# SuperScientificSoftwareLaboratory/TileSpMV

Measured on AMD Instinct MI355X. Metric: fp64 SpMV GFLOP/s (y = A*x, tiled format), higher is better.
Workload: dtype f64; 1 GPU; laplacian4096; rows=16777216, cols=16777216, nnz=83869696, partition=tile-row blocks, nnz-balanced, 1 rank(s), y_combine=none, tiles=5234176, x_panel_merge=0, x_slice_passes=0

## Files before the change

include/tilespmv.h:

```cpp
#ifndef TILESPMV_H_
#define TILESPMV_H_

#include <stddef.h>
#include <stdint.h>

#ifdef __cplusplus
extern "C" {
#endif

#ifndef MAT_VAL_TYPE
#define MAT_VAL_TYPE double
#endif
#ifndef MAT_PTR_TYPE
#define MAT_PTR_TYPE int
#endif

#define TILESPMV_BLOCK_SIZE 16
#define TILESPMV_COO_NNZ_TH 12
#define TILESPMV_PREFETCH_SMEM_TH 4

enum {
    TILESPMV_FMT_CSR = 0,
    TILESPMV_FMT_COO = 1,
    TILESPMV_FMT_ELL = 2,
// ... 87 lines not shown
                      const MAT_PTR_TYPE *csrRowPtr, const int *csrColIdx, const MAT_VAL_TYPE *csrVal,
                      const char *source_mtx);
int tilespmv_csr_load(const char *path, int *m, int *n, MAT_PTR_TYPE *nnz, int *isSymmetric,
                      MAT_PTR_TYPE **csrRowPtr, int **csrColIdx, MAT_VAL_TYPE **csrVal,
                      const char *source_mtx);
int mmio_allinone_cached(int *m, int *n, MAT_PTR_TYPE *nnz, int *isSymmetric, MAT_PTR_TYPE **csrRowPtr,
                         int **csrColIdx, MAT_VAL_TYPE **csrVal, char *filename, const char *cache_path,
                         int *from_cache);
int tilespmv_mtx_write(const char *path, int m, int n, MAT_PTR_TYPE nnz, const MAT_PTR_TYPE *csrRowPtr,
                       const int *csrColIdx, const MAT_VAL_TYPE *csrVal);


void call_tilespmv_hip(char *filename, Tile_matrix *matrix, int *ptroffset1, int *ptroffset2,
                       int rowblkblock, unsigned int *blkcoostylerowidx,
                       int *blkcoostylerowidx_colstart, int *blkcoostylerowidx_colstop, int rowA,
                       int colA, MAT_PTR_TYPE nnzA, MAT_PTR_TYPE *csrRowPtrA, int *csrColIdxA,
                       MAT_VAL_TYPE *csrValA, MAT_VAL_TYPE alpha, MAT_VAL_TYPE *x,
                       MAT_VAL_TYPE *y, MAT_VAL_TYPE *y_golden);

#define TILESPMV_Y_SHARDED 0
#define TILESPMV_Y_ALLGATHER 1
#define TILESPMV_Y_ALLREDUCE 2
int call_tilespmv_hip_multi(char *filename, Tile_matrix *matrix, int *ptroffset1, int *ptroffset2,
                             int rowblkblock, unsigned int *blkcoostylerowidx,
                             int *blkcoostylerowidx_colstart, int *blkcoostylerowidx_colstop,
                             int rowA, int colA, MAT_PTR_TYPE nnzA, MAT_PTR_TYPE *csrRowPtrA,
                             int *csrColIdxA, MAT_VAL_TYPE *csrValA, MAT_VAL_TYPE alpha,
                             MAT_VAL_TYPE *x, MAT_VAL_TYPE *y, MAT_VAL_TYPE *y_golden, int ngpus,
                             const int *device_ids, int y_combine_mode);

typedef struct tilespmv_plan tilespmv_plan;

#define TILESPMV_COO_AUTO 0
#define TILESPMV_COO_IN_TILE 1
#define TILESPMV_COO_FALLBACK 2

#define TILESPMV_DENSE_AUTO 0
#define TILESPMV_DENSE_MFMA 1
#define TILESPMV_DENSE_VALU 2

#define TILESPMV_KERNEL_AUTO 0
#define TILESPMV_KERNEL_DIRECT 1
#define TILESPMV_KERNEL_STREAM 2

#define TILESPMV_KNOB_DEFAULT (-1)
typedef struct {
    unsigned size;
    int coo_mode;
    int dense_mode;
    int kernel;
    int tilerow_begin;
    int tilerow_end;
    int autotune;
    int entry_mode;
    int entry_ordered;
    int strip_cost;
    int split_above;
    int split_cap;
    int xcd_remap;
    int xcd_chunk;
    int csr_split;
    int fix_inline;
    int coo_cost;
    int coo_heavy_min;
    int coo_piece;
    int strip_even;
    int wg_strips;
    int x_window;
    int x_stride1;
    int x_stride2;
    int mv_native;
    int mv_xcd_chunk;
    int lds_pad;
    int y_store;
    int desc_dict;
    int nt_stream;
    int x_panel_kb;
    int x_panel_merge;
    int placement_tries;
    int x_slice_passes;
    int deterministic;
    int absorb;
    int value_narrow;
    int reserved[1];
} tilespmv_plan_options;
void tilespmv_plan_options_init(tilespmv_plan_options *opts);
const char *tilespmv_plan_options_layout(void);

int tilespmv_plan_create(tilespmv_plan **plan, const Tile_matrix *matrix, int rowA, int colA,
                         MAT_PTR_TYPE nnzA, const tilespmv_plan_options *opts);
void tilespmv_plan_destroy(tilespmv_plan *plan);

int Tile_create_device(Tile_matrix *matrix, int rowA, int colA, MAT_PTR_TYPE nnzA, const MAT_PTR_TYPE *csrRowPtrA,
                       const int *csrColIdxA, const MAT_VAL_TYPE *csrValA, unsigned flags);
int tilespmv_plan_create_from_csr(tilespmv_plan **plan, int rowA, int colA, MAT_PTR_TYPE nnzA, const MAT_PTR_TYPE *csrRowPtrA,
                                  const int *csrColIdxA, const MAT_VAL_TYPE *csrValA, unsigned create_flags,
                                  const tilespmv_plan_options *opts);
int tilespmv_plan_create_from_device_csr(tilespmv_plan **plan, int rowA, int colA, MAT_PTR_TYPE nnzA, const MAT_PTR_TYPE *d_csrRowPtrA,
                                         const int *d_csrColIdxA, const MAT_VAL_TYPE *d_csrValA, unsigned create_flags,
                                         const tilespmv_plan_options *opts);

#define TILESPMV_ERR_NO_VALUE_MAP (-4)
int tilespmv_plan_update_values(tilespmv_plan *plan, const MAT_VAL_TYPE *d_csrVal, void *stream);

int tilespmv_plan_spmv(tilespmv_plan *plan, const MAT_VAL_TYPE *d_x, MAT_VAL_TYPE *d_y,
                       void *stream);

int tilespmv_plan_spmv_n(tilespmv_plan *plan, const MAT_VAL_TYPE *d_x, MAT_VAL_TYPE *d_y, void *stream, int count);

#define TILESPMV_MAX_NVEC 8
int tilespmv_plan_spmm(tilespmv_plan *plan, const MAT_VAL_TYPE *d_X, MAT_VAL_TYPE *d_Y, int nvec,
                       void *stream);
double tilespmv_plan_time_spmm(tilespmv_plan *plan, const MAT_VAL_TYPE *d_X, MAT_VAL_TYPE *d_Y,
                               int nvec, void *stream, int warmup, int reps);
int tilespmv_plan_reserve_spmm(tilespmv_plan *plan, int nvec);

int tilespmv_plan_layout_digest(const Tile_matrix *matrix, int rowA, int colA, MAT_PTR_TYPE nnzA,
                                const tilespmv_plan_options *opts, unsigned long long *digest,
                                long long *info );

enum {
    TILESPMV_STAGE_COUNT_ROWS = 0,
    TILESPMV_STAGE_CHOOSE = 1,
    TILESPMV_STAGE_CUT = 2,
    TILESPMV_STAGE_EMIT = 3,
    TILESPMV_STAGE_ORDER = 4,
    TILESPMV_STAGE_ENCODE = 5,
    TILESPMV_STAGE_ENTRIES = 6,
    TILESPMV_STAGE_FINISH = 7,
    TILESPMV_STAGE_COUNT = 8
};
int tilespmv_plan_layout_stages(const Tile_matrix *matrix, int rowA, int colA, MAT_PTR_TYPE nnzA,
                                const tilespmv_plan_options *opts, unsigned long long *stage_digests,
                                long long *info );

enum {
    TILESPMV_INFO_DEVICE_BYTES = 0,
    TILESPMV_INFO_STREAM_BYTES = 1,
    TILESPMV_INFO_NNZ = 2,
    TILESPMV_INFO_ROWS = 3,
    TILESPMV_INFO_TILES = 4,
    TILESPMV_INFO_COO_MODE = 5,
    TILESPMV_INFO_DENSE_MODE = 6,
    TILESPMV_INFO_KERNEL = 7,
    TILESPMV_INFO_NUM_TASKS = 8,
    TILESPMV_INFO_NUM_SPLIT_ROWS = 9,
    TILESPMV_INFO_FALLBACK_NNZ = 10,
    TILESPMV_INFO_BUILD_US = 11,
    TILESPMV_INFO_UPLOAD_US = 12,
    TILESPMV_INFO_ENTRY_MODE = 13,
    TILESPMV_INFO_ENTRY_ORDERED = 14,
    TILESPMV_INFO_STRIP_COST = 15,
    TILESPMV_INFO_WG_STRIPS = 16,
    TILESPMV_INFO_LIST_ENTRIES = 17,
    TILESPMV_INFO_DERIVED_UNITS = 18,
    TILESPMV_INFO_BRICK_ORDER = 19,
    TILESPMV_INFO_DESC_BYTES = 20,
    TILESPMV_INFO_NT_STREAM = 21,
    TILESPMV_INFO_UNIT_VALUE_BYTES = 22,
    TILESPMV_INFO_RETIRED_23 = 23,
    TILESPMV_INFO_PLACEMENT_TRIES = 24,
    TILESPMV_INFO_RETIRED_25 = 25,
    TILESPMV_INFO_X_PANELS = 26,
    TILESPMV_INFO_X_PANEL_MERGE = 27,
    TILESPMV_INFO_SCATTERED_ENTRIES = 28,
    TILESPMV_INFO_X_SLICE_PASSES = 29,
    TILESPMV_INFO_CSR_FORM = 30,
    TILESPMV_INFO_TIMED_CHOICES_US = 31,
    TILESPMV_INFO_DEVICE_BUILD = 32,
    TILESPMV_INFO_TILE_CREATE_US = 33,
    TILESPMV_INFO_VALUE_MAP_BYTES = 34,
    TILESPMV_INFO_COUNT = 35
};
void tilespmv_plan_info(const tilespmv_plan *plan, long long *out );
long long tilespmv_plan_stream_digests(const tilespmv_plan *plan, unsigned long long *out , long long max_streams);

double tilespmv_plan_time(tilespmv_plan *plan, const MAT_VAL_TYPE *d_x, MAT_VAL_TYPE *d_y,
                          void *stream, int warmup, int reps);

double tilespmv_plan_time_reference_style(tilespmv_plan *plan, const MAT_VAL_TYPE *d_x, MAT_VAL_TYPE *d_y,
                                          void *stream, int reps);

void tilespmv_partition_tilerows(const Tile_matrix *matrix, int nparts, int *bounds);

int tilespmv_sizeof_value(void);

int tilespmv_reorder_rcm(int n, const MAT_PTR_TYPE *csrRowPtr, const int *csrColIdx, int *perm );
int tilespmv_csr_permute(int n, const MAT_PTR_TYPE *csrRowPtr, const int *csrColIdx, const MAT_VAL_TYPE *csrVal, const int *perm,
                         MAT_PTR_TYPE *outRowPtr , int *outColIdx, MAT_VAL_TYPE *outVal);
long long tilespmv_csr_bandwidth(int n, const MAT_PTR_TYPE *csrRowPtr, const int *csrColIdx);
int tilespmv_permute_vector(const MAT_VAL_TYPE *d_in, MAT_VAL_TYPE *d_out, const int *d_perm, long long n, int scatter, void *stream);

int tilespmv_csr_transpose(int rowA, int colA, const MAT_PTR_TYPE *csrRowPtr, const int *csrColIdx, const MAT_VAL_TYPE *csrVal ,
                           MAT_PTR_TYPE *rowPtrT , int *colIdxT, MAT_VAL_TYPE *valT , int *srcT );
int tilespmv_csr_transpose_device(int rowA, int colA, const MAT_PTR_TYPE *d_csrRowPtr, const int *d_csrColIdx, const MAT_VAL_TYPE *d_csrVal ,
                                  MAT_PTR_TYPE *d_rowPtrT, int *d_colIdxT, MAT_VAL_TYPE *d_valT , int *d_srcT , void *stream);

typedef struct tilespmv_cg tilespmv_cg;
typedef struct { unsigned size; int iterations; int status; double rr; double bb; } tilespmv_cg_state;
#define TILESPMV_CG_RUNNING 0
#define TILESPMV_CG_CONVERGED 1
#define TILESPMV_CG_MAXITER 2
#define TILESPMV_CG_BREAKDOWN 3
int tilespmv_cg_create(tilespmv_cg **cg, tilespmv_plan *plan, const MAT_VAL_TYPE *d_dinv );
void tilespmv_cg_destroy(tilespmv_cg *cg);
int tilespmv_cg_begin(tilespmv_cg *cg, const MAT_VAL_TYPE *d_b, MAT_VAL_TYPE *d_x, void *stream);
int tilespmv_cg_iterate(tilespmv_cg *cg, MAT_VAL_TYPE *d_x, int count, void *stream);
int tilespmv_cg_state_read(tilespmv_cg *cg, void *stream, tilespmv_cg_state *out);
int tilespmv_cg_solve(tilespmv_cg *cg, const MAT_VAL_TYPE *d_b, MAT_VAL_TYPE *d_x, double rtol, int maxiter, int check_every, void *stream, tilespmv_cg_state *out);
int tilespmv_csr_diagonal_device(int rows, const MAT_PTR_TYPE *d_csrRowPtr, const int *d_csrColIdx, const MAT_VAL_TYPE *d_csrVal, MAT_VAL_TYPE *d_out, int invert, void *stream);

typedef struct tilespmv_cg_multi tilespmv_cg_multi;
int tilespmv_cg_multi_create(tilespmv_cg_multi **cg, tilespmv_plan *plan, int nvec, const MAT_VAL_TYPE *d_dinv );
void tilespmv_cg_multi_destroy(tilespmv_cg_multi *cg);
int tilespmv_cg_multi_begin(tilespmv_cg_multi *cg, const MAT_VAL_TYPE *d_B, MAT_VAL_TYPE *d_X, void *stream);
int tilespmv_cg_multi_iterate(tilespmv_cg_multi *cg, MAT_VAL_TYPE *d_X, int count, void *stream);
int tilespmv_cg_multi_state_read(tilespmv_cg_multi *cg, void *stream, tilespmv_cg_state *out );
int tilespmv_cg_multi_solve(tilespmv_cg_multi *cg, const MAT_VAL_TYPE *d_B, MAT_VAL_TYPE *d_X, double rtol, int maxiter, int check_every, void *stream,
                            tilespmv_cg_state *out );

typedef struct tilespmv_cgls tilespmv_cgls;
typedef struct { unsigned size; int iterations; int status; double nn; double nn0; double rr; double bb; } tilespmv_cgls_state;
int tilespmv_cgls_create(tilespmv_cgls **ls, tilespmv_plan *plan_A, tilespmv_plan *plan_AT, const MAT_VAL_TYPE *d_cinv );
void tilespmv_cgls_destroy(tilespmv_cgls *ls);
int tilespmv_cgls_begin(tilespmv_cgls *ls, const MAT_VAL_TYPE *d_b, MAT_VAL_TYPE *d_x, double damp, void *stream);
int tilespmv_cgls_iterate(tilespmv_cgls *ls, MAT_VAL_TYPE *d_x, int count, void *stream);
int tilespmv_cgls_state_read(tilespmv_cgls *ls, void *stream, tilespmv_cgls_state *out);
int tilespmv_cgls_solve(tilespmv_cgls *ls, const MAT_VAL_TYPE *d_b, MAT_VAL_TYPE *d_x, double damp, double rtol, int maxiter, int check_every, void *stream,
                        tilespmv_cgls_state *out);
int tilespmv_csr_row_sqnorms_device(int rows, const MAT_PTR_TYPE *d_rowPtr, const int *d_src , const MAT_VAL_TYPE *d_val, MAT_VAL_TYPE *d_out, int invert,
                                    void *stream);

typedef struct tilespmv_bicgstab tilespmv_bicgstab;
int tilespmv_bicgstab_create(tilespmv_bicgstab **s, tilespmv_plan *plan, const MAT_VAL_TYPE *d_dinv );
void tilespmv_bicgstab_destroy(tilespmv_bicgstab *s);
int tilespmv_bicgstab_begin(tilespmv_bicgstab *s, const MAT_VAL_TYPE *d_b, MAT_VAL_TYPE *d_x, void *stream);
int tilespmv_bicgstab_iterate(tilespmv_bicgstab *s, MAT_VAL_TYPE *d_x, int count, void *stream);
int tilespmv_bicgstab_state_read(tilespmv_bicgstab *s, void *stream, tilespmv_cg_state *out);
int tilespmv_bicgstab_solve(tilespmv_bicgstab *s, const MAT_VAL_TYPE *d_b, MAT_VAL_TYPE *d_x, double rtol, int maxiter, int check_every, void *stream,
                            tilespmv_cg_state *out);

typedef struct tilespmv_minres tilespmv_minres;
int tilespmv_minres_create(tilespmv_minres **s, tilespmv_plan *plan, const MAT_VAL_TYPE *d_minv );
// ... 17 lines not shown
```

tilespmv_amd/_lib.py:

```python
import ctypes as C
import os
import subprocess

import numpy as np

from .tile_matrix import TileMatrixF32, TileMatrixF64

_ROOT = os.path.dirname(os.path.abspath(__file__))
_I = C.POINTER(C.c_int)
_U = C.POINTER(C.c_uint)
_CACHE = {}

INFO_NAMES = ["device_bytes", "stream_bytes", "nnz", "rows", "tiles", "coo_mode", "dense_mode", "kernel",
              "num_tasks", "num_split_rows", "fallback_nnz", "build_us", "upload_us", "entry_mode", "entry_ordered", "strip_cost",
              "wg_strips", "list_entries", "derived_units", "brick_order", "desc_bytes", "nt_stream", "unit_value_bytes", "retired_23", "placement_tries", "retired_25", "x_panels", "x_panel_merge", "scattered_entries", "x_slice_passes", "csr_form", "timed_choices_us", "device_build", "tile_create_us",
              "value_map_bytes"]


KNOB_DEFAULT = -1
KNOB_NAMES = ["entry_mode", "entry_ordered", "strip_cost", "split_above", "split_cap", "xcd_remap", "xcd_chunk", "csr_split", "fix_inline",
              "coo_cost", "coo_heavy_min", "coo_piece", "strip_even", "wg_strips", "x_window", "x_stride1", "x_stride2", "mv_native", "mv_xcd_chunk", "lds_pad", "y_store", "desc_dict", "nt_stream", "x_panel_kb", "x_panel_merge", "placement_tries", "x_slice_passes", "deterministic", "absorb", "value_narrow"]


class PlanOptions(C.Structure):
    _fields_ = ([("size", C.c_uint), ("coo_mode", C.c_int), ("dense_mode", C.c_int), ("kernel", C.c_int),
                 ("tilerow_begin", C.c_int), ("tilerow_end", C.c_int), ("autotune", C.c_int)] +
                [(k, C.c_int) for k in KNOB_NAMES] + [("reserved", C.c_int * 1)])

    def __init__(self, coo_mode=0, dense_mode=0, kernel=0, tilerow_begin=0, tilerow_end=0, autotune=False, **knobs):
        super().__init__()
        self.size = C.sizeof(PlanOptions)
        self.coo_mode, self.dense_mode, self.kernel = coo_mode, dense_mode, kernel
        self.tilerow_begin, self.tilerow_end, self.autotune = tilerow_begin, tilerow_end, 1 if autotune else 0
        for k in KNOB_NAMES:
            setattr(self, k, KNOB_DEFAULT)
        for i in range(len(self.reserved)):
            self.reserved[i] = KNOB_DEFAULT
        for k, v in knobs.items():
            if k not in KNOB_NAMES:
                raise TypeError("unknown plan knob %r (known: %s)" % (k, ", ".join(KNOB_NAMES)))
            setattr(self, k, int(v))


class CGState(C.Structure):
    _fields_ = [("size", C.c_uint), ("iterations", C.c_int), ("status", C.c_int), ("rr", C.c_double), ("bb", C.c_double)]

    def __init__(self):
        super().__init__()
        self.size = C.sizeof(CGState)


class CGLSState(C.Structure):
    _fields_ = [("size", C.c_uint), ("iterations", C.c_int), ("status", C.c_int), ("nn", C.c_double), ("nn0", C.c_double), ("rr", C.c_double), ("bb", C.c_double)]

    def __init__(self):
        super().__init__()
        self.size = C.sizeof(CGLSState)


def lib_path(dtype):
    suf = "f64" if np.dtype(dtype) == np.float64 else "f32"
    return os.path.join(_ROOT, "lib", "libtilespmv_%s%s.so" % (suf, os.environ.get("TILESPMV_LIB_VARIANT", "")))


def build(verbose=False):
    cmd = ["make", "-C", os.path.join(_ROOT, "csrc"), "-j8", "all"]
    res = subprocess.run(cmd, stdout=subprocess.PIPE, stderr=subprocess.STDOUT, text=True)
    if verbose or res.returncode != 0:
        print(res.stdout)
    if res.returncode != 0:
        raise RuntimeError("building tilespmv_amd/csrc failed")
    return [lib_path(np.float64), lib_path(np.float32)]


def load(dtype=np.float64):
    dtype = np.dtype(dtype)
    if dtype in _CACHE:
        return _CACHE[dtype]
    path = lib_path(dtype)
    if not os.path.exists(path):
        raise RuntimeError("HIP extension %s is missing — run `python -c 'import __graft_entry__ as g; g.build()'` "
                           "(or `make -C tilespmv_amd/csrc`); there is no CPU fallback" % path)
    lib = C.CDLL(path, mode=C.RTLD_GLOBAL if False else C.RTLD_LOCAL)
    vt = C.c_double if dtype == np.float64 else C.c_float
    TM = TileMatrixF64 if dtype == np.float64 else TileMatrixF32
    VP, TP = C.POINTER(vt), C.POINTER(TM)
    assert lib.tilespmv_sizeof_value() == dtype.itemsize
    lib.Tile_create.argtypes = [TP, C.c_int, C.c_int, C.c_int, _I, _I, VP]
    lib.Tile_create.restype = None
    lib.Tile_create_ex.argtypes = [TP, C.c_int, C.c_int, C.c_int, _I, _I, VP, C.c_uint]
    lib.Tile_create_ex.restype = None
    lib.Tile_create_device.argtypes = [TP, C.c_int, C.c_int, C.c_int, _I, _I, VP, C.c_uint]
    lib.Tile_create_device.restype = C.c_int
    lib.tilespmv_plan_create_from_csr.argtypes = [C.POINTER(C.c_void_p), C.c_int, C.c_int, C.c_int, _I, _I, VP, C.c_uint, C.POINTER(PlanOptions)]
    lib.tilespmv_plan_create_from_csr.restype = C.c_int
    lib.tilespmv_plan_create_from_device_csr.argtypes = [C.POINTER(C.c_void_p), C.c_int, C.c_int, C.c_int, C.c_void_p, C.c_void_p, C.c_void_p, C.c_uint, C.POINTER(PlanOptions)]
    lib.tilespmv_plan_create_from_device_csr.restype = C.c_int
    lib.tilespmv_plan_update_values.argtypes = [C.c_void_p, C.c_void_p, C.c_void_p]
    lib.tilespmv_plan_update_values.restype = C.c_int
    lib.tilespmv_plan_stream_digests.argtypes = [C.c_void_p, C.POINTER(C.c_ulonglong), C.c_longlong]
    lib.tilespmv_plan_stream_digests.restype = C.c_longlong
    lib.Tile_destroy.argtypes = [TP]
    lib.Tile_destroy.restype = None
    lib.tilespmv_cpu.argtypes = [TP, _I, _I, _I, C.POINTER(_U), C.POINTER(_I), C.POINTER(_I), C.c_int, C.c_int, C.c_int,
# ... 161 lines not shown
```

tilespmv_amd/csrc/hip_kernels.hip:

```cpp
#include <hip/hip_runtime.h>

#include "hip_plan.h"
#include "plan_tile_ops.h"
#include "hip_units_kernel.h"

namespace tilespmv {


typedef double v4d __attribute__((ext_vector_type(4)));
typedef float v4f __attribute__((ext_vector_type(4)));

constexpr int GROUPS_PER_BLOCK = 16;
#ifndef TILESPMV_STREAM_MIN_WAVES
#define TILESPMV_STREAM_MIN_WAVES 1
#endif

__device__ __forceinline__ int nibble_of(const unsigned char *__restrict__ base, int p)
{
    const unsigned b = base[p >> 1];
    return (p & 1) ? (int)(b & 15u) : (int)(b >> 4);
}

__device__ __forceinline__ void mfma_dense_tile(const val_t *__restrict__ tile, const val_t *xseg, int lane, val_t *out16)
{
// ... 1046 lines not shown
    switch (nvec) {
    case 2: return launch_mv<2>(P, S, DN, xcd_chunk, entries_pass, slab_rows, X, Y, st);
    case 4: return launch_mv<4>(P, S, DN, xcd_chunk, entries_pass, slab_rows, X, Y, st);
    case 8: return launch_mv<8>(P, S, DN, xcd_chunk, entries_pass, slab_rows, X, Y, st);
    default: return hipErrorInvalidValue;
    }
}

__global__ __launch_bounds__(256) void k_rows_to_columns(const val_t *__restrict__ X, int nvec, long long n, long long ld, val_t *__restrict__ XT)
{
    const long long i = (long long)blockIdx.x * 256 + threadIdx.x;
    if (i >= n) return;
    for (int j = 0; j < nvec; j++) XT[j * ld + i] = X[i * nvec + j];
}
__global__ __launch_bounds__(256) void k_columns_to_rows(const val_t *__restrict__ YT, int nvec, long long row0, long long rows, long long ld, val_t *__restrict__ Y)
{
    const long long i = (long long)blockIdx.x * 256 + threadIdx.x;
    if (i >= rows) return;
    for (int j = 0; j < nvec; j++) Y[(row0 + i) * nvec + j] = YT[j * ld + i];
}
__global__ __launch_bounds__(256) void k_permute_vector(const val_t *__restrict__ in, val_t *__restrict__ out, const int *__restrict__ perm, long long n, int scatter)
{
    const long long i = (long long)blockIdx.x * 256 + threadIdx.x;
    if (i >= n) return;
    const long long p = perm[i];
    if (scatter) out[p] = in[i]; else out[i] = in[p];
}
hipError_t launch_permute_vector(const val_t *in, val_t *out, const int *perm, long long n, int scatter, hipStream_t st)
{
    if (n > 0) hipLaunchKernelGGL(k_permute_vector, dim3((unsigned)((n + 255) / 256)), dim3(256), 0, st, in, out, perm, n, scatter);
    return hipGetLastError();
}

hipError_t launch_rows_to_columns(const val_t *X, int nvec, long long n, long long ld, val_t *XT, hipStream_t st)
{
    if (n > 0) hipLaunchKernelGGL(k_rows_to_columns, dim3((unsigned)((n + 255) / 256)), dim3(256), 0, st, X, nvec, n, ld, XT);
    return hipGetLastError();
}
hipError_t launch_columns_to_rows(const val_t *YT, int nvec, long long row0, long long rows, long long ld, val_t *Y, hipStream_t st)
{
    if (rows > 0) hipLaunchKernelGGL(k_columns_to_rows, dim3((unsigned)((rows + 255) / 256)), dim3(256), 0, st, YT, nvec, row0, rows, ld, Y);
    return hipGetLastError();
}

__global__ __launch_bounds__(256) void k_pair_values(const val_t *__restrict__ src, val_t *__restrict__ dst, const int4 *__restrict__ map, int ntasks, int narrow)
{
    const int G = narrow ? UNIT_GROUP_NARROW : UNIT_GROUP;
    float *__restrict__ dstn = reinterpret_cast<float *>(dst);
    unsigned short *__restrict__ dsth = reinterpret_cast<unsigned short *>(dst);
    for (int t = blockIdx.x; t < ntasks; t += gridDim.x) {
        const int4 m = map[t];
        const long long so = (long long)m.x * 16, dofs = (long long)m.y * 16;
        for (int i = threadIdx.x; i < m.z * 16; i += 256) {
            const int j = i >> 4, r = i & 15;
            const long long at = dofs + (long long)(j / G * G) * 16 + G * r + (j % G);
            if (narrow == 2) dsth[at] = value_half_bits((double)src[so + i]);
            else if (narrow) dstn[at] = (float)src[so + i];
            else dst[at] = src[so + i];
        }
    }
}

hipError_t launch_pair_values(const val_t *src, val_t *dst, const int4 *map, int ntasks, int narrow)
{
    if (ntasks > 0) hipLaunchKernelGGL(k_pair_values, dim3((unsigned)std::min(ntasks, 1 << 20)), dim3(256), 0, nullptr, src, dst, map, ntasks, narrow);
    return hipGetLastError();
}

hipError_t launch_tiles_stream(const DevPlan &P, const DevStream &S, const DevDense &DN, bool dense_mfma, int entry_mode, int wg_strips, int lds_pad_bytes, int xcd_remap, int xcd_chunk,
                               const val_t *x, val_t *y, hipStream_t st)
{
    if (S.ntasks > 0) {
        const int xc = xcd_remap == 2 ? xcd_chunk : 0;
#define TSPMV_KN(W, CD) hipLaunchKernelGGL((k_units<TILESPMV_UB, W, 16, CD, true, false, false, true>), dim3((unsigned)((S.ntasks + 15) / 16)), dim3(256), (size_t)lds_pad_bytes, st, S, P.rowA, P.colA, xc, P.partial, x, y)
#define TSPMV_K(W, B, CD, NTS, PL, WD) hipLaunchKernelGGL((k_units<TILESPMV_UB, W, B, CD, NTS, PL, WD>), dim3((unsigned)((S.ntasks + B - 1) / B)), dim3(16 * B), (size_t)lds_pad_bytes, st, S, P.rowA, P.colA, xc, P.partial, x, y)
#define TSPMV_NTS(W, B, CD, PL, WD) do { if (S.nt_stream) TSPMV_K(W, B, CD, true, PL, WD); else TSPMV_K(W, B, CD, false, PL, WD); } while (0)
#define TSPMV_FORM_(W, B, L) do { \
            if (S.pooled) { if (S.ucol) L(W, B, false, true, true); else if (S.pdict) L(W, B, true, true, false); else L(W, B, false, true, false); } \
            else if (S.cb_bits > 0) L(W, B, true, false, false); else L(W, B, false, false, false); } while (0)
#define TSPMV_PLAIN(W, B, CD, PL, WD) TSPMV_K(W, B, CD, false, PL, WD)
#define TSPMV_FORM(W, B) TSPMV_FORM_(W, B, TSPMV_NTS)
#define TSPMV_FORM_SMALL(W, B) TSPMV_FORM_(W, B, TSPMV_PLAIN)
        const bool small_grid = entry_mode != 2 && !S.nt_stream && (S.ntasks + 15) / 16 < SMALL_GRID_WORKGROUPS;
#if !defined(TILESPMV_F32)
        if (S.uval_narrow == 2) {
            const hipError_t eh = launch_units_half(P, S, entry_mode, wg_strips, lds_pad_bytes, xc, x, y, st);
            if (eh != hipSuccess) return eh;
        } else if (S.uval_narrow) {
            if (S.pooled || !S.nt_stream || entry_mode == 1 || wg_strips != 16) return hipErrorInvalidValue;
            if (entry_mode == 2) { if (S.cb_bits > 0) TSPMV_KN(2, true); else TSPMV_KN(2, false); }
            else { if (S.cb_bits > 0) TSPMV_KN(0, true); else TSPMV_KN(0, false); }
        } else
#endif
        if (small_grid) { if (entry_mode == 1) TSPMV_FORM_SMALL(1, 8); else TSPMV_FORM_SMALL(0, 8); }
        else if (entry_mode == 1) TSPMV_FORM_SMALL(1, 16);
        else if (entry_mode == 2 && wg_strips == 32 && !S.pooled) {
            if (S.cb_bits > 0) TSPMV_NTS(2, 32, true, false, false); else TSPMV_NTS(2, 32, false, false, false);
        }
        else if (entry_mode == 2) TSPMV_FORM(2, 16);
        else TSPMV_FORM(0, 16);
#undef TSPMV_FORM_SMALL
#undef TSPMV_FORM
#undef TSPMV_PLAIN
#undef TSPMV_FORM_
#undef TSPMV_NTS
#undef TSPMV_K
#undef TSPMV_KN
    }
    hipError_t e = launch_tiles_direct(P, dense_mfma, true, false, x, y, st);
    if (e != hipSuccess) return e;
    e = launch_dense_mfma(DN, S.nt_stream != 0, P.rowA, P.colA, P.partial, x, y, st);
    if (e != hipSuccess) return e;
    if (P.nfix_late > 0) {
        DevPlan Q = P;
        Q.fix = P.fix_late; Q.nfix = P.nfix_late;
        hipLaunchKernelGGL(k_fixup_split, dim3((Q.nfix + GROUPS_PER_BLOCK - 1) / GROUPS_PER_BLOCK), dim3(256), 0, st, Q, y);
    }
    if (S.slice_passes > 0 && S.x_panels > 1 && S.ntasks > 0) return launch_entry_slices(S, P.rowA, x, y, st);
    if (S.panel_merge > 0 && S.x_panels > S.panel_merge && S.ntasks > 0) return launch_entry_panels(P, S, xcd_remap, xcd_chunk, x, y, st);
    return hipGetLastError();
}

}
```

tilespmv_amd/csrc/hip_plan.h:

```cpp
#pragma once
#include <cstdint>

#include "host_util.h"

namespace tilespmv {

constexpr unsigned DESC_FMT_MASK = 7u;
constexpr unsigned DESC_FMT_NOP = 7u;
constexpr unsigned DESC_EOR = 8u;
constexpr int DESC_P1_SHIFT = 4;
constexpr int DESC_P2_SHIFT = 12;

#if defined(TILESPMV_F32)
struct ERec { unsigned v, w; };
#else
struct ERec { unsigned lo, hi, w; };
#endif
constexpr int ECHUNK = 64;
constexpr int SMALL_GRID_WORKGROUPS = 128;
constexpr int FB_DEST_BITS = 11;

struct Task {
    int tile_begin, tile_end;
    long long val_off;
// ... 21 lines not shown
    const unsigned *f_base;
    int f_nblk;
    int f_ordered;
    int f_row0;
    int f_rows;
};

constexpr int FB_ROWS = 2048;
constexpr int FB_CAP = 6144;
constexpr int STRIP_MAX_ROWS = 8;
constexpr unsigned UNIT_EOR = 1u;
constexpr int UNIT_ROW_SHIFT = 1;
constexpr unsigned UNIT_ROWUNIT = 16u;
constexpr int UNIT_SHIFT_SHIFT = 29;
constexpr int ABSORB_SHIFT_MIN = -3, ABSORB_SHIFT_MAX = 3;
constexpr unsigned UNIT_DERIVED_CODE = 4u;
constexpr int UNIT_GROUP = 16 / (int)sizeof(val_t);
constexpr int UNIT_GROUP_NARROW = 4;
constexpr long long NT_STREAM_MIN_BYTES = 400ll << 20;
constexpr int DICT_MAX_BITS = 10;
constexpr int UNIT_FLAG_SHIFT = 24;

struct UDesc { unsigned w0, n0, n1; };

constexpr int POOL_KR_SHIFT = 28;
constexpr unsigned POOL_BASE_MASK = (1u << POOL_KR_SHIFT) - 1u;
constexpr int POOL_WORD_KR_SHIFT = 30;
__host__ __device__ inline int pool_word_base_bits(int npatterns)
{
    int ib = 1;
    while ((1 << ib) < npatterns) ib++;
    return POOL_WORD_KR_SHIFT - ib;
}
constexpr int POOL_MIN_FILL = sizeof(val_t) == 8 ? 12 : 10;
#ifndef TILESPMV_POOL_STRIP_ROWS
#define TILESPMV_POOL_STRIP_ROWS 4
#endif
constexpr int POOL_STRIP_ROWS = TILESPMV_POOL_STRIP_ROWS;
struct URow { unsigned r0, r1; };
constexpr unsigned POOL_WIDE_WINDOW = 256;
constexpr double POOL_WIDE_MAX_LINES = 3.5;

struct STask {
    int unit_begin, unit_end;
    int coo_begin, coo_end;
    int row;
    int partial;
    unsigned nounit_mask;
    int nrows;
};

struct DevStream {
    const UDesc *udesc;
    const URow *urow;
    const uint4 *ucol;
    const uint4 *pdict;
    int pooled;
    const val_t *uval;
    const val_t *cval;
    const int *ccol;
    const unsigned char *crow;
    const STask *task;
    int ntasks;
    int coo_heavy_min;
    int coo_ordered;
    int y_streaming;
    const int4 *wg_coo;
    const ERec *grec;
    const unsigned *gbase;
    int dest_bits;
    const uint4 *udict;
    int cb_bits;
    int nt_stream;
    int uval_narrow;
    const int *panel_off;
    int x_panels;
    int panel_merge;
    int n_groups;
    int slice_passes;
    int slice_ct;
    const UDesc *udesc_cb;
    const FixRow *ifix;
    unsigned *ifix_count;
};

struct DenseRow { int row, tile_begin, tile_end, partial; };
__host__ __device__ constexpr int dense_slot(int r, int c)
{
    return sizeof(val_t) == 8 ? ((c & 3) >> 1) * 128 + ((c >> 2) * 16 + r) * 2 + (c & 1) : ((c >> 2) * 16 + r) * 4 + (c & 3);
}

struct DevDense {
    const int *cb;
    const val_t *val;
    const DenseRow *rows;
    int nrows;
};

inline void tile_stream_sizes(int fmt, int p1, int p2, int *nv, int *ni)
{
    switch (fmt) {
    case TILESPMV_FMT_CSR: *nv = p1; *ni = 16 + (p1 + 1) / 2; break;
    case TILESPMV_FMT_COO: *nv = p1; *ni = p1; break;
    case TILESPMV_FMT_ELL: *nv = 16 * p1; *ni = 8 * p1; break;
    case TILESPMV_FMT_HYB: *nv = 16 * p1 + p2; *ni = 8 * p1 + p2; break;
    case TILESPMV_FMT_DNS: *nv = 256; *ni = 0; break;
    case TILESPMV_FMT_DNSROW: *nv = 16 * p1; *ni = p1; break;
    case TILESPMV_FMT_DNSCOL: *nv = 16 * p1; *ni = p1; break;
    default: *nv = 0; *ni = 0; break;
    }
}

hipError_t launch_units_half(const DevPlan &P, const DevStream &S, int entry_mode, int wg_strips, int lds_pad_bytes, int xcd_chunk, const val_t *x, val_t *y, hipStream_t st);

}
```

tilespmv_amd/csrc/hip_plan.hip:

```cpp
#include <type_traits>

#include "hip_plan_internal.h"
#include "hip_plan_device.h"
#include "tile_fields.h"

namespace tilespmv {
hipError_t launch_permute_vector(const val_t *in, val_t *out, const int *perm, long long n, int scatter, hipStream_t st);

hipError_t launch_tiles_direct(const DevPlan &P, bool dense_mfma, bool accumulate, bool fixup, const val_t *x, val_t *y, hipStream_t st);
hipError_t launch_tiles_stream(const DevPlan &P, const DevStream &S, const DevDense &DN, bool dense_mfma, int entry_mode, int wg_strips, int lds_pad_bytes, int xcd_remap, int xcd_chunk,
                               const val_t *x, val_t *y, hipStream_t st);
hipError_t launch_fallback(const DevPlan &P, const val_t *x, val_t *y, hipStream_t st);
hipError_t launch_tiles_stream_mv(const DevPlan &P, const DevStream &S, const DevDense &DN, int nvec, int xcd_chunk, bool entries_pass, int slab_rows, const val_t *X, val_t *Y,
                                  hipStream_t st);
hipError_t launch_rows_to_columns(const val_t *X, int nvec, long long n, long long ld, val_t *XT, hipStream_t st);
hipError_t launch_columns_to_rows(const val_t *YT, int nvec, long long row0, long long rows, long long ld, val_t *Y, hipStream_t st);

static Knobs resolve_knobs(const tilespmv_plan_options *opts)
{
    tilespmv_plan_options o;
    tilespmv_plan_options_init(&o);
    if (opts && opts->size >= sizeof(unsigned)) memcpy(&o, opts, std::min<size_t>(opts->size, sizeof(o)));
    o.size = (unsigned)sizeof(o);
    auto pick = [](int opt, const char *env, int dflt) { return opt != TILESPMV_KNOB_DEFAULT ? opt : env_int(env, dflt); };
    auto pinned = [](int opt, const char *env) { return opt != TILESPMV_KNOB_DEFAULT || getenv(env) != nullptr; };
    Knobs k{};
    k.coo_mode = o.coo_mode > 0 ? o.coo_mode : env_int("TILESPMV_COO_MODE", 0);
    k.dense_mode = o.dense_mode > 0 ? o.dense_mode : env_int("TILESPMV_DENSE_MODE", 0);
    k.kernel = o.kernel > 0 ? o.kernel : env_int("TILESPMV_KERNEL", 0);
    k.tilerow_begin = o.tilerow_begin; k.tilerow_end = o.tilerow_end;
    k.autotune = (o.autotune > 0 || env_int("TILESPMV_AUTOTUNE", 0) != 0) ? 1 : 0;
    k.entry_mode = pick(o.entry_mode, "TILESPMV_WAVE_COO", -1);
    k.entry_ordered = pick(o.entry_ordered, "TILESPMV_COO_ORDERED", -1);
    k.strip_cost = pick(o.strip_cost, "TILESPMV_STRIP_COST", 0);
    k.split_above = pick(o.split_above, "TILESPMV_SPLIT_ABOVE", 2400);
    k.split_cap = pick(o.split_cap, "TILESPMV_SPLIT_CAP", 4800);
    k.xcd_remap = pick(o.xcd_remap, "TILESPMV_XCD_REMAP", 2) ? 2 : 0;
    k.xcd_chunk = std::max(1, pick(o.xcd_chunk, "TILESPMV_XCD_CHUNK", 32));
    k.csr_split = pick(o.csr_split, "TILESPMV_CSR_SPLIT", -1);
    k.fix_inline = pick(o.fix_inline, "TILESPMV_FIX_INLINE", 1);
    k.coo_cost = pick(o.coo_cost, "TILESPMV_COO_COST", 4);
    k.coo_heavy_min = std::max(0, pick(o.coo_heavy_min, "TILESPMV_COO_HEAVY_MIN", 32));
    k.coo_piece = pick(o.coo_piece, "TILESPMV_COO_PIECE", 0);
    k.strip_even = pick(o.strip_even, "TILESPMV_STRIP_EVEN", 4);
    k.wg_strips = pick(o.wg_strips, "TILESPMV_WG_STRIPS", -1);
    k.x_window = pick(o.x_window, "TILESPMV_X_WINDOW", -1);
    k.x_stride1 = pick(o.x_stride1, "TILESPMV_X_STRIDE1", 0);
    k.x_stride2 = pick(o.x_stride2, "TILESPMV_X_STRIDE2", 0);
    k.lds_pad = pick(o.lds_pad, "TILESPMV_LDS_PAD", -1);
    k.y_store = pick(o.y_store, "TILESPMV_Y_STORE", -1);
    k.mv_native = pick(o.mv_native, "TILESPMV_MV_NATIVE", -1);
    k.mv_xcd_chunk = pick(o.mv_xcd_chunk, "TILESPMV_MV_XCD_CHUNK", -1);
    k.desc_dict = pick(o.desc_dict, "TILESPMV_DESC_DICT", -1);
    k.nt_stream = pick(o.nt_stream, "TILESPMV_NT_STREAM", -1);
    k.placement_tries = pick(o.placement_tries, "TILESPMV_PLACEMENT_TRIES", -1);
    k.x_panel_kb = pick(o.x_panel_kb, "TILESPMV_X_PANEL_KB", -1);
    k.x_panel_merge = pick(o.x_panel_merge, "TILESPMV_X_PANEL_MERGE", -1);
    k.x_slice_passes = pick(o.x_slice_passes, "TILESPMV_X_SLICE_PASSES", -1);
    k.absorb = pick(o.absorb, "TILESPMV_ABSORB", -1); if (k.absorb < 0 || k.absorb > 2) k.absorb = 1;
    k.value_narrow = pick(o.value_narrow, "TILESPMV_VALUE_NARROW", -1);
    k.deterministic = pick(o.deterministic, "TILESPMV_DETERMINISTIC", 0) > 0 ? 1 : 0;
    if (k.deterministic) {
        if (k.placement_tries < 0) k.placement_tries = 1;
        if (k.x_panel_merge < 0) k.x_panel_merge = 0;
        if (k.x_slice_passes < 0) k.x_slice_passes = 0;
        k.autotune = 0;
        k.entry_ordered = 1; k.x_slice_passes = 0;
    }
    k.xcd_from_caller = pinned(o.xcd_remap, "TILESPMV_XCD_REMAP") || pinned(o.xcd_chunk, "TILESPMV_XCD_CHUNK");
    k.entry_from_caller = pinned(o.entry_mode, "TILESPMV_WAVE_COO");
    k.strip_from_caller = o.strip_cost > 0 || env_int("TILESPMV_STRIP_COST", 0) > 0;
    k.autotune_log = getenv("TILESPMV_AUTOTUNE_LOG");
    k.verbose = getenv("TILESPMV_PLAN_VERBOSE") != nullptr;
    k.placement_force = env_int("TILESPMV_PLACEMENT_FORCE", 0) != 0;
    k.encode_check = env_int("TILESPMV_ENCODE_CHECK", 0) != 0;
    k.encode_on_host = env_int("TILESPMV_ENCODE_ON_HOST", 0) != 0;
    return k;
}

}

using namespace tilespmv;

template <class F>
static void for_each_plan_pointer(tilespmv_plan *plan, F f)
{
    DevPlan &D = plan->dev; DevStream &S = plan->st; DevDense &N = plan->dn;
    auto v = [&](auto &p) {
        const void *q = (const void *)p;
        f(q);
        p = (std::remove_reference_t<decltype(p)>)const_cast<void *>(q);
    };
    for (const void **slot : plan->uploaded_slots) f(*slot);
    (void)D; (void)N;
    v(D.partial); v(S.udesc_cb); v(S.ifix_count);
}

static void retry_placement(tilespmv_plan *plan, int tries, const Knobs &K)
{
    plan->info[TILESPMV_INFO_PLACEMENT_TRIES] = 1;
    if (tries <= 1 || plan->arena_blocks.empty()) return;
    typedef std::vector<std::pair<void *, size_t>> Blocks;
    val_t *dx = nullptr, *dy = nullptr;
    const size_t nx = (size_t)plan->dev.colA + 16, ny = (size_t)plan->dev.rowA + 16;
    if (hipMalloc((void **)&dx, nx * sizeof(val_t)) != hipSuccess) { (void)hipGetLastError(); return; }
    if (hipMalloc((void **)&dy, ny * sizeof(val_t)) != hipSuccess) { (void)hipGetLastError(); (void)hipFree(dx); return; }
    { std::vector<val_t> ones(nx, (val_t)1); (void)hipMemcpy(dx, ones.data(), nx * sizeof(val_t), hipMemcpyHostToDevice); }
    auto rebase = [&](const Blocks &from, const Blocks &to) {
        for_each_plan_pointer(plan, [&](const void *&p) {
            if (!p) return;
            for (size_t i = 0; i < from.size(); i++) {
                const char *b0 = (const char *)from[i].first;
                if ((const char *)p >= b0 && (const char *)p < b0 + from[i].second) { p = (const char *)to[i].first + ((const char *)p - b0); return; }
            }
        });
    };
    auto show = [&](int t, double ms, const Blocks &bl) {
        if (!K.verbose) return;
        fprintf(stderr, "tilespmv: placement %d: %.4f ms  blocks at", t, ms);
        for (auto &b : bl) fprintf(stderr, " %p(+%zu MB)", b.first, b.second >> 20);
        fprintf(stderr, "\n");
    };
    std::vector<Blocks> cand{plan->arena_blocks};
    std::vector<double> ms{tilespmv_plan_time(plan, dx, dy, nullptr, 3, 5)};
    show(1, ms[0], cand[0]);
    size_t at = 0, best = 0;
    for (int t = 2; t <= tries && ms[0] > 0; t++) {
        Blocks fresh;
        bool ok = true;
        for (auto &b : cand[0]) {
            void *nb = nullptr;
            {
                size_t mem_free = 0, mem_total = 0;
                if (hipMemGetInfo(&mem_free, &mem_total) != hipSuccess) { (void)hipGetLastError(); ok = false; break; }
                if (mem_free < b.second + ((size_t)512 << 20)) { ok = false; break; }
            }
            if (plan->block_alloc(&nb, b.second, true) != 0) { ok = false; break; }
            fresh.push_back({nb, b.second});
            if (hipMemcpy(nb, cand[at][fresh.size() - 1].first, b.second, hipMemcpyDeviceToDevice) != hipSuccess) { (void)hipGetLastError(); ok = false; break; }
        }
        if (!ok) { for (auto &b : fresh) plan->block_free(b.first); break; }
        rebase(cand[at], fresh);
        cand.push_back(fresh); at = cand.size() - 1;
// ... 10 lines not shown
        if (slow_confirmed > 0 && ms[best] < 0.91 * slow_confirmed) break;
        if (ms.size() >= 5 && hi < 1.015 * lo) break;
    }
    if (at != best) rebase(cand[at], cand[best]);
    {
        int dangling = 0;
        for_each_plan_pointer(plan, [&](const void *&p) {
            if (!p) return;
            for (size_t i = 0; i < cand.size(); i++) {
                if (i == best) continue;
                for (auto &b : cand[i]) if ((const char *)p >= (const char *)b.first && (const char *)p < (const char *)b.first + b.second) dangling++;
            }
        });
        if (dangling) { fprintf(stderr, "tilespmv: internal error: %d plan pointers left in a dropped placement\n", dangling); abort(); }
    }
    for (size_t i = 0; i < cand.size(); i++) {
        if (i == best) continue;
        for (auto &b : cand[i]) plan->block_free(b.first);
    }
    if (best != 0) plan->arena_blocks = cand[best];
    plan->arena_at = nullptr; plan->arena_left = 0;
    if (K.verbose) fprintf(stderr, "tilespmv: placement %zu of %zu kept (%.4f ms; first %.4f)\n", best + 1, cand.size(), ms[best], ms[0]);
    (void)hipFree(dx); (void)hipFree(dy);
}

extern "C" {

int tilespmv_device_count(void)
{
    int n = 0;
    if (hipGetDeviceCount(&n) != hipSuccess) return 0;
    return n;
}

int tilespmv_sizeof_value(void) { return (int)sizeof(val_t); }

int tilespmv_permute_vector(const MAT_VAL_TYPE *d_in, MAT_VAL_TYPE *d_out, const int *d_perm, long long n, int scatter, void *stream)
{
    if (n < 0 || (n > 0 && (!d_in || !d_out || !d_perm)) || d_in == d_out) return (int)hipErrorInvalidValue;
    return (int)tilespmv::launch_permute_vector(d_in, d_out, d_perm, n, scatter, (hipStream_t)stream);
}
const char *tilespmv_version(void) { return "tilespmv-mi355x 0.1 (gfx950)"; }

void tilespmv_partition_tilerows(const Tile_matrix *T, int nparts, int *bounds)
{
    const long long total = T->blknnz[T->tilenum];
    bounds[0] = 0;
    int bi = 0;
    for (int p = 1; p < nparts; p++) {
        const long long want = total * p / nparts;
        while (bi < T->tilem && T->blknnz[T->tile_ptr[bi]] < want) bi++;
        bounds[p] = std::max(bi, bounds[p - 1]);
    }
    bounds[nparts] = T->tilem;
}

void tilespmv_plan_destroy(tilespmv_plan *plan)
{
    if (!plan) return;
    for (void *p : plan->allocs) (void)hipFree(p);
    delete plan;
}

static int plan_create_one(tilespmv_plan **out, const Tile_matrix *T, int rowA, int colA, MAT_PTR_TYPE nnzA, const Knobs &K, const DevTile *DT = nullptr);

void tilespmv_plan_options_init(tilespmv_plan_options *o)
{
    memset(o, 0, sizeof(*o));
    o->size = (unsigned)sizeof(*o);
    int *knob = &o->entry_mode;
    const int n = (int)((sizeof(*o) - offsetof(tilespmv_plan_options, entry_mode)) / sizeof(int));
    for (int i = 0; i < n; i++) knob[i] = TILESPMV_KNOB_DEFAULT;
}

const char *tilespmv_plan_options_layout(void)
{
    static const std::string s = [] {
        std::string o;
#define TSPMV_F(f) o += std::string(o.empty() ? "" : ",") + #f + ":" + std::to_string(offsetof(tilespmv_plan_options, f));
        TSPMV_F(size) TSPMV_F(coo_mode) TSPMV_F(dense_mode) TSPMV_F(kernel) TSPMV_F(tilerow_begin) TSPMV_F(tilerow_end) TSPMV_F(autotune)
        TSPMV_F(entry_mode) TSPMV_F(entry_ordered) TSPMV_F(strip_cost) TSPMV_F(split_above) TSPMV_F(split_cap) TSPMV_F(xcd_remap) TSPMV_F(xcd_chunk)
        TSPMV_F(csr_split) TSPMV_F(fix_inline) TSPMV_F(coo_cost) TSPMV_F(coo_heavy_min) TSPMV_F(coo_piece) TSPMV_F(strip_even) TSPMV_F(wg_strips)
        TSPMV_F(x_window) TSPMV_F(x_stride1) TSPMV_F(x_stride2) TSPMV_F(mv_native) TSPMV_F(mv_xcd_chunk) TSPMV_F(lds_pad) TSPMV_F(y_store)
        TSPMV_F(desc_dict) TSPMV_F(nt_stream) TSPMV_F(x_panel_kb) TSPMV_F(x_panel_merge) TSPMV_F(placement_tries) TSPMV_F(x_slice_passes) TSPMV_F(deterministic) TSPMV_F(absorb) TSPMV_F(value_narrow) TSPMV_F(reserved)
#undef TSPMV_F
        return o;
    }();
    return s.c_str();
}

static int plan_create_tuned(tilespmv_plan **out, const Tile_matrix *T, int rowA, int colA, MAT_PTR_TYPE nnzA, const Knobs &Kc, const DevTile *DT);
int tilespmv_plan_create(tilespmv_plan **out, const Tile_matrix *T, int rowA, int colA, MAT_PTR_TYPE nnzA,
                         const tilespmv_plan_options *opts)
{
    const Knobs Kc = resolve_knobs(opts);
    if (!Kc.autotune) return plan_create_one(out, T, rowA, colA, nnzA, Kc);
    return plan_create_tuned(out, T, rowA, colA, nnzA, Kc, nullptr);
}
static int plan_create_tuned(tilespmv_plan **out, const Tile_matrix *T, int rowA, int colA, MAT_PTR_TYPE nnzA, const Knobs &Kc, const DevTile *DT)
{
    Knobs K0 = Kc;
    if (Kc.placement_tries < 0) K0.placement_tries = 1;
    *out = nullptr;
    const int tilem = T->tilem;
    const int tr0 = std::max(0, K0.tilerow_begin), tr1 = (K0.tilerow_end <= 0 || K0.tilerow_end > tilem) ? tilem : K0.tilerow_end;
    bool has_dense = false;
    for (int t = T->tile_ptr[tr0]; t < T->tile_ptr[tr1] && !has_dense; t++) has_dense = T->Format[t] == TILESPMV_FMT_DNS;
    const bool has_extracted = !DT && T->new_coocount[T->tile_ptr[tr1]] > T->new_coocount[T->tile_ptr[tr0]];
    val_t *dx = nullptr, *dy = nullptr;
    if (hipMalloc((void **)&dx, ((size_t)colA + 16) * sizeof(val_t)) != hipSuccess) return -3;
    if (hipMalloc((void **)&dy, ((size_t)rowA + 16) * sizeof(val_t)) != hipSuccess) { (void)hipFree(dx); return -3; }
    {
        std::vector<val_t> ones((size_t)colA + 16, (val_t)1);
        (void)hipMemcpy(dx, ones.data(), ones.size() * sizeof(val_t), hipMemcpyHostToDevice);
    }
    tilespmv_plan *best = nullptr;
    double best_ms = 0;
    std::string log = "{\"rows\": " + std::to_string(rowA) + ", \"cols\": " + std::to_string(colA) + ", \"nnz\": " + std::to_string((long long)nnzA) +
                      ", \"value_bytes\": " + std::to_string(sizeof(val_t)) + ", \"candidates\": [";
    bool first = true;
    auto try_one = [&](const Knobs &cand, const char *label) {
        tilespmv_plan *p = nullptr;
        if (plan_create_one(&p, T, rowA, colA, nnzA, cand, DT) != 0 || !p) return;
        const double ms = tilespmv_plan_time(p, dx, dy, nullptr, 3, 12);
        char buf[512];
        snprintf(buf, sizeof(buf), "%s{\"label\": \"%s\", \"coo_mode\": %d, \"dense_mode\": %d, \"entry_mode\": %d, \"ordered\": %lld, \"strip_cost\": %lld, \"tasks\": %lld, \"ms\": %.5f}",
                 first ? "" : ", ", label, p->coo_mode, p->dense_mode, p->entry_mode, p->info[TILESPMV_INFO_ENTRY_ORDERED], p->info[TILESPMV_INFO_STRIP_COST],
                 p->info[TILESPMV_INFO_NUM_TASKS], ms);
        log += buf; first = false;
        bool take = ms > 0 && (!best || ms < best_ms * 0.985);
        double ms_c = ms;
        if (take && best) {
            double hold = best_ms, chal = ms;
            for (int rep = 0; rep < 2; rep++) {
                const double h = tilespmv_plan_time(best, dx, dy, nullptr, 2, 20), c = tilespmv_plan_time(p, dx, dy, nullptr, 2, 20);
                if (h > 0) hold = rep ? std::min(hold, h) : h;
                if (c > 0) chal = rep ? std::min(chal, c) : c;
            }
            take = chal < hold * 0.985;
            best_ms = hold; ms_c = chal;
            char b2[96];
            snprintf(b2, sizeof(b2), ", {\"label\": \"confirm\", \"holder_ms\": %.5f, \"challenger_ms\": %.5f}", hold, chal);
            log += b2;
        }
        if (take) { tilespmv_plan_destroy(best); best = p; best_ms = ms_c; }
        else tilespmv_plan_destroy(p);
    };
    const int coo_cands[2] = {TILESPMV_COO_IN_TILE, TILESPMV_COO_FALLBACK}, dns_cands[2] = {TILESPMV_DENSE_MFMA, TILESPMV_DENSE_VALU};
    try_one(K0, "default");
    const tilespmv_plan *dflt = best;
    const int d_coo = dflt ? dflt->coo_mode : 0, d_dns = dflt ? dflt->dense_mode : 0, d_entry = dflt ? dflt->entry_mode : 0;
    const long long d_cost = dflt ? dflt->info[TILESPMV_INFO_STRIP_COST] : 400, d_ord = dflt ? dflt->info[TILESPMV_INFO_ENTRY_ORDERED] : 1;
    const bool coo_var = K0.coo_mode == TILESPMV_COO_AUTO && has_extracted, dns_var = K0.dense_mode == TILESPMV_DENSE_AUTO && has_dense;
    for (int ci = 0; ci < (coo_var ? 2 : 1); ci++)
        for (int di = 0; di < (dns_var ? 2 : 1); di++) {
            Knobs cand = K0;
            if (coo_var) cand.coo_mode = coo_cands[ci];
            if (dns_var) cand.dense_mode = dns_cands[di];
            if ((!coo_var || cand.coo_mode == d_coo) && (!dns_var || cand.dense_mode == d_dns)) continue;
            try_one(cand, "coo/dense mode");
        }
    if (best && best->kernel == TILESPMV_KERNEL_STREAM && best->coo_mode == TILESPMV_COO_IN_TILE && !K0.entry_from_caller && !K0.strip_from_caller) {
        Knobs cand = K0;
        cand.coo_mode = best->coo_mode; cand.dense_mode = best->dense_mode;
        const bool may_unorder = K0.entry_ordered != 1;
        for (int em = 0; em <= 2; em++) {
            if (em == d_entry && !(em == 2)) continue;
            Knobs c2 = cand; c2.entry_mode = em;
            if (em == 2) {
                if (d_entry != 2 || d_ord == 0) { c2.entry_ordered = 1; try_one(c2, "entry mode 2, ordered"); }
                if (may_unorder && (d_entry != 2 || d_ord == 1)) { c2.entry_ordered = 0; try_one(c2, "entry mode 2, unordered"); }
            } else try_one(c2, em == 0 ? "entry mode 0" : "entry mode 1");
        }
        const int w_entry = best->entry_mode; const long long w_ord = best->info[TILESPMV_INFO_ENTRY_ORDERED], w_cost = best->info[TILESPMV_INFO_STRIP_COST];
        for (long long c : {w_cost / 2, w_cost * 2}) {
            if (c < 100 || c > 3200 || c == d_cost) continue;
            Knobs c2 = cand; c2.entry_mode = w_entry; c2.strip_cost = (int)c;
            if (w_entry == 2) c2.entry_ordered = w_ord ? 1 : 0;
            try_one(c2, "strip size");
        }
        auto with_winner = [&](Knobs c2) {
            c2.entry_mode = best->entry_mode; c2.strip_cost = (int)best->info[TILESPMV_INFO_STRIP_COST];
            if (best->entry_mode == 2) c2.entry_ordered = best->info[TILESPMV_INFO_ENTRY_ORDERED] ? 1 : 0;
            return c2;
        };
        if (K0.csr_split < 0)
            for (int form = 1; form <= 3; form++) {
                if (form == (int)best->info[TILESPMV_INFO_CSR_FORM]) continue;
                Knobs c2 = cand; c2.csr_split = form;
                try_one(c2, form == 1 ? "CSR tiles split" : form == 2 ? "CSR tiles pooled" : "CSR tiles pooled, wide windows");
            }
        if (K0.x_window < 0 && best->info[TILESPMV_INFO_BRICK_ORDER]) { Knobs c2 = with_winner(cand); c2.csr_split = (int)best->info[TILESPMV_INFO_CSR_FORM]; c2.x_window = 0; try_one(c2, "no brick order"); }
        if (K0.wg_strips < 0 && best->entry_mode == 2 && best->wg_strips == 16 && !best->pooled) {
            Knobs c2 = with_winner(cand); c2.wg_strips = 32; c2.x_window = 0;
            try_one(c2, "32 strips per workgroup");
            c2.strip_cost = 6400; try_one(c2, "32 strips per workgroup, strips of 6400");
        }
    }
    log += "], \"xcd_maps\": [";
    if (best && best->kernel == TILESPMV_KERNEL_STREAM && !K0.xcd_from_caller) {
        const int maps[3][2] = {{best->xcd_remap, best->xcd_chunk}, {0, best->xcd_chunk}, {2, 8}};
        int pick = 0;
        double pick_ms = 0;
        for (int k = 0; k < 3; k++) {
            best->xcd_remap = maps[k][0]; best->xcd_chunk = maps[k][1];
            const double ms = tilespmv_plan_time(best, dx, dy, nullptr, 3, 20);
            char buf[128];
            snprintf(buf, sizeof(buf), "%s{\"remap\": %d, \"chunk\": %d, \"ms\": %.5f}", k ? ", " : "", maps[k][0], maps[k][1], ms);
            log += buf;
            if (ms > 0 && (k == 0 || ms < pick_ms * 0.985)) { pick = k; pick_ms = ms; }
        }
        best->xcd_remap = maps[pick][0]; best->xcd_chunk = maps[pick][1];
        best_ms = std::min(best_ms, pick_ms);
    }
    log += "], \"stream_policy\": [";
    if (best && best->kernel == TILESPMV_KERNEL_STREAM && K0.nt_stream < 0 && best->entry_mode != 1 && !best->st.uval_narrow) {
        const int rule = best->st.nt_stream;
        double ms2[2] = {0, 0};
        for (int k = 0; k < 2; k++) {
            best->st.nt_stream = k ? 1 - rule : rule;
            ms2[k] = tilespmv_plan_time(best, dx, dy, nullptr, 3, 20);
            char buf[96];
            snprintf(buf, sizeof(buf), "%s{\"nontemporal\": %d, \"ms\": %.5f}", k ? ", " : "", best->st.nt_stream, ms2[k]);
            log += buf;
        }
        const bool flip = ms2[1] > 0 && ms2[1] < ms2[0] * 0.985;
        best->st.nt_stream = flip ? 1 - rule : rule;
        best->info[TILESPMV_INFO_NT_STREAM] = best->st.nt_stream;
        if (ms2[flip ? 1 : 0] > 0) best_ms = std::min(best_ms, ms2[flip ? 1 : 0]);
    }
    if (best) {
        char buf[512];
        snprintf(buf, sizeof(buf), "], \"choice\": {\"coo_mode\": %d, \"dense_mode\": %d, \"entry_mode\": %d, \"ordered\": %lld, \"strip_cost\": %lld, \"xcd_remap\": %d, \"xcd_chunk\": %d, \"nontemporal\": %d, \"ms\": %.5f}}",
                 best->coo_mode, best->dense_mode, best->entry_mode, best->info[TILESPMV_INFO_ENTRY_ORDERED], best->info[TILESPMV_INFO_STRIP_COST], best->xcd_remap, best->xcd_chunk, best->st.nt_stream, best_ms);
        log += buf;
        if (K0.autotune_log) {
            if (FILE *f = fopen(K0.autotune_log, "a")) { fprintf(f, "%s\n", log.c_str()); fclose(f); }
        }
    }
    (void)hipFree(dx); (void)hipFree(dy);
    if (!best) return -4;
    if (Kc.placement_tries < 0 && best->info[TILESPMV_INFO_DEVICE_BYTES] >= (1ll << 30)) {
        const double t0p = now_us();
        retry_placement(best, 8, Kc);
        best->info[TILESPMV_INFO_BUILD_US] += (long long)(now_us() - t0p);
        best->info[TILESPMV_INFO_TIMED_CHOICES_US] += (long long)(now_us() - t0p);
    }
    *out = best;
    return 0;
}

static void calibrate_panels(tilespmv_plan *plan, int colA, bool verbose)
{
    DevStream &S = plan->st;
    val_t *dx = nullptr, *dy = nullptr;
    const size_t nx = (size_t)plan->dev.colA + 16, ny = (size_t)plan->dev.rowA + 16;
    S.panel_merge = 0; S.slice_passes = 0;
    if (hipMalloc((void **)&dx, nx * sizeof(val_t)) != hipSuccess) { (void)hipGetLastError(); return; }
    if (hipMalloc((void **)&dy, ny * sizeof(val_t)) != hipSuccess) { (void)hipGetLastError(); (void)hipFree(dx); return; }
    { std::vector<val_t> ones(nx, (val_t)1); (void)hipMemcpy(dx, ones.data(), nx * sizeof(val_t), hipMemcpyHostToDevice); }
    const double t_base = tilespmv_plan_time(plan, dx, dy, nullptr, 3, 8);
    double best = t_base; int best_m = 0, best_s = 0;
    const double x_mb = (double)colA * sizeof(val_t) / (1 << 20), panel_mb = x_mb / S.x_panels;
    int last = 0;
    for (double mb : {4.0, 8.0, 16.0}) {
        const int m = std::max(1, (int)(mb / std::max(panel_mb, 1e-9) + 0.5));
        if (m == last || m >= S.x_panels) continue;
        last = m;
        S.panel_merge = m;
        const double t = tilespmv_plan_time(plan, dx, dy, nullptr, 2, 8);
        if (verbose) fprintf(stderr, "tilespmv: column panels: %d passes of %.1f MB of x -> %.4f ms (plain %.4f)\n", (S.x_panels + m - 1) / m, m * panel_mb, t, t_base);
        if (t > 0 && t < best) { best = t; best_m = m; best_s = 0; }
    }
    S.panel_merge = 0;
    if (plan->slice_calibrate)
        for (int passes : {1, 2, 4}) {
            const double slice_mb = x_mb / (8.0 * passes);
            if (slice_mb > 8.5 || (passes > 1 && slice_mb < 0.9) || 8 * passes > 2 * S.x_panels) continue;
            S.slice_passes = passes; S.slice_ct = slice_trip_records(plan->list_records, S.n_groups, passes);
            const double t = tilespmv_plan_time(plan, dx, dy, nullptr, 2, 8);
            if (verbose) fprintf(stderr, "tilespmv: column slices on XCDs: %d pass(es), %.1f MB of x per XCD -> %.4f ms (plain %.4f)\n", passes, slice_mb, t, t_base);
            if (t > 0 && t < best) { best = t; best_m = 0; best_s = passes; }
        }
    const bool keep = best < 0.97 * t_base;
    S.slice_passes = keep ? best_s : 0;
    S.slice_ct = slice_trip_records(plan->list_records, S.n_groups, std::max(1, S.slice_passes));
    S.panel_merge = keep ? best_m : 0;
    if (verbose) fprintf(stderr, "tilespmv: entry lists: %s\n", S.slice_passes ? "column slices on XCDs" : S.panel_merge ? "column panels" : "plain launch");
    (void)hipFree(dx); (void)hipFree(dy);
}

static int plan_create_one(tilespmv_plan **out, const Tile_matrix *T, int rowA, int colA, MAT_PTR_TYPE nnzA, const Knobs &K, const DevTile *DT)
{
    (void)nnzA;
    *out = nullptr;
    const double t_create0 = now_us();
    if (!K.dry && tilespmv_device_count() <= 0) {
        fprintf(stderr, "tilespmv: no HIP device visible — the GPU path has no CPU fallback\n");
        return -1;
    }
    const Knobs &o = K;
    const int tilem = T->tilem, tilen = T->tilen;
    const int tr0 = std::max(0, o.tilerow_begin), tr1 = (o.tilerow_end <= 0 || o.tilerow_end > tilem) ? tilem : o.tilerow_end;
    const int ntr = std::max(0, tr1 - tr0);
    const int sv = (int)sizeof(val_t);

    auto *plan = new tilespmv_plan();
    plan->dry = K.dry;
    if (!K.dry && hipGetDevice(&plan->device) != hipSuccess) { fprintf(stderr, "tilespmv: hipGetDevice failed\n"); delete plan; return -1; }

    const int t_begin = T->tile_ptr[tr0], t_end = T->tile_ptr[tr1];
// ... 172 lines not shown
                for (int sft = P0[r]; sft < P0[r + 1]; sft += FB_CAP) f_blk.push_back(make_int4(r, -1, sft - base, std::min(sft + FB_CAP, P0[r + 1]) - base));
                r++;
                continue;
            }
            int e = r, cnt = 0;
            while (e < rows && e - r < FB_ROWS && (P0[e + 1] - P0[e]) <= FB_CAP && (e == r || cnt + (P0[e + 1] - P0[e]) <= cap)) { cnt += P0[e + 1] - P0[e]; e++; }
            while (e > r + 1 && P0[e] == P0[e - 1]) e--;
            f_blk.push_back(make_int4(r, e - r, P0[r] - base, P0[e] - base));
            r = e;
        }
        std::vector<std::vector<ERec>> blk_rec(f_blk.size());
        std::vector<std::vector<unsigned>> blk_base(f_blk.size());
        std::atomic<int> bad(0);
        parallel_chunks((int64_t)f_blk.size(), 16, [&](int64_t b0, int64_t b1, int) {
            std::vector<std::pair<unsigned long long, int>> key;
            std::vector<PEnt> ents;
            for (int64_t b = b0; b < b1; b++) {
                const int4 k = f_blk[(size_t)b];
                key.clear();
                if (k.y < 0) {
                    for (int q = k.z; q < k.w; q++) key.push_back({((unsigned long long)(unsigned)T->deferredcoo_colidx[base + q] << 32) | (unsigned)(q - k.z), 0});
                } else {
                    for (int rr = k.x; rr < k.x + k.y; rr++)
                        for (int q = P0[rr] - base; q < P0[rr + 1] - base; q++)
                            key.push_back({((unsigned long long)(unsigned)T->deferredcoo_colidx[base + q] << 32) | (unsigned)(q - k.z), rr - k.x});
                }
                std::sort(key.begin(), key.end());
                ents.resize(key.size());
                for (size_t i = 0; i < key.size(); i++) {
                    const int q = k.z + (int)(key[i].first & 0xFFFFFFFFull);
                    ents[i] = PEnt{(unsigned)T->deferredcoo_colidx[base + q], (unsigned)key[i].second, T->deferredcoo_val[base + q]};
                }
                if (!pack_list(ents, FB_DEST_BITS, blk_rec[(size_t)b], blk_base[(size_t)b], K.dry)) bad++;
            }
        });
        if (bad.load()) { fprintf(stderr, "tilespmv: internal error: %d packed fallback lists do not decode to their entries\n", bad.load()); rc = -6; }
        long long at = 0;
        for (size_t b = 0; b < f_blk.size(); b++) {
            f_blk[b].z = (int)at; f_blk[b].w = (int)(at + (long long)blk_rec[b].size());
            at = (at + (long long)blk_rec[b].size() + ECHUNK - 1) / ECHUNK * ECHUNK;
            if (at > INT32_MAX - ECHUNK) { fprintf(stderr, "tilespmv: shard too large for 32-bit entry ids\n"); rc = -2; break; }
        }
        if (rc == 0) {
            f_rec.assign((size_t)at, make_erec((val_t)0, 0u));
            f_base.assign((size_t)(at / ECHUNK), 0u);
            parallel_chunks((int64_t)f_blk.size(), 64, [&](int64_t b0, int64_t b1, int) {
                for (int64_t b = b0; b < b1; b++) {
                    if (!blk_rec[(size_t)b].empty()) memcpy(&f_rec[(size_t)f_blk[(size_t)b].z], blk_rec[(size_t)b].data(), blk_rec[(size_t)b].size() * sizeof(ERec));
                    if (!blk_base[(size_t)b].empty()) memcpy(&f_base[(size_t)(f_blk[(size_t)b].z / ECHUNK)], blk_base[(size_t)b].data(), blk_base[(size_t)b].size() * sizeof(unsigned));
                }
            });
        }
    }

    rc |= plan->upload(fix.data(), fix.size(), &D.fix);
    if (npartial > 0) {
        void *p = nullptr;
        if (K.dry) { }
        else if (hipMalloc(&p, (size_t)npartial * 16 * sizeof(val_t) * TILESPMV_MAX_NVEC) != hipSuccess) rc = -3;
        else { plan->allocs.push_back(p); plan->arena_blocks.push_back({p, (size_t)npartial * 16 * sizeof(val_t) * TILESPMV_MAX_NVEC}); D.partial = (val_t *)p; }
    }
    if (!f_blk.empty()) {
        rc |= plan->upload(f_rec.data(), f_rec.size(), &D.f_rec);
        rc |= plan->upload(f_base.data(), f_base.size(), &D.f_base);
        rc |= plan->upload(f_blk.data(), f_blk.size(), &D.f_blk);
        D.f_nblk = (int)f_blk.size();
        const int ordered_env = K.entry_ordered;
        D.f_ordered = ordered_env >= 0 ? ordered_env != 0 : f_blk.size() >= 2048;
    }
    if (rc) { tilespmv_plan_destroy(plan); return rc; }
    D.nfix = (int)fix.size();
    D.rowA = std::min<long long>(rowA, (long long)tr1 * 16); D.colA = colA;
    D.f_row0 = row0; D.f_rows = rows;
    plan->matrix_rows = rowA;

    long long *I = plan->info;
    I[TILESPMV_INFO_NNZ] = span(T->tile_nnz, DT ? DT->T.tile_nnz : nullptr, t_begin, t_end);
    I[TILESPMV_INFO_ROWS] = rows;
    I[TILESPMV_INFO_TILES] = t_end - t_begin;
    I[TILESPMV_INFO_COO_MODE] = coo_mode; I[TILESPMV_INFO_DENSE_MODE] = dense_mode; I[TILESPMV_INFO_KERNEL] = plan->kernel;
    I[TILESPMV_INFO_NUM_TASKS] = n_tasks; I[TILESPMV_INFO_NUM_SPLIT_ROWS] = (long long)fix.size();
    I[TILESPMV_INFO_FALLBACK_NNZ] = f_nnz;
    I[TILESPMV_INFO_UNIT_VALUE_BYTES] = plan->st.uval_narrow == 2 ? 2 : plan->st.uval_narrow ? 4 : sv;
    if (plan->kernel != TILESPMV_KERNEL_STREAM) { I[TILESPMV_INFO_ENTRY_ORDERED] = 1; I[TILESPMV_INFO_STRIP_COST] = target; }
    I[TILESPMV_INFO_BUILD_US] = (long long)(now_us() - t_create0) - I[TILESPMV_INFO_UPLOAD_US];
    I[TILESPMV_INFO_STREAM_BYTES] = model_bytes + (long long)colA * sv + (long long)rows * sv +
                                    (f_nnz ? (long long)f_rec.size() * (long long)sizeof(ERec) + (long long)f_base.size() * 4 + 2LL * sv * rows + (long long)f_blk.size() * 16 : 0);
    if (!K.dry) {
        const int tries = K.placement_tries >= 0 ? K.placement_tries : (I[TILESPMV_INFO_DEVICE_BYTES] >= (1ll << 30) ? 8 : 1);
        const double t0p = now_us();
        retry_placement(plan, tries, K);
        I[TILESPMV_INFO_BUILD_US] += (long long)(now_us() - t0p);
        if (tries > 1 && !plan->arena_blocks.empty()) I[TILESPMV_INFO_TIMED_CHOICES_US] += (long long)(now_us() - t0p);
    }
    if (!K.dry && plan->panel_calibrate) {
        const double t0c = now_us();
        calibrate_panels(plan, colA, K.verbose);
        I[TILESPMV_INFO_BUILD_US] += (long long)(now_us() - t0c);
        I[TILESPMV_INFO_TIMED_CHOICES_US] += (long long)(now_us() - t0c);
    }
    if (plan->st.panel_merge > 0) {
        const int m = plan->st.panel_merge, passes = (plan->st.x_panels + m - 1) / m;
        I[TILESPMV_INFO_X_PANELS] = passes;
        I[TILESPMV_INFO_STREAM_BYTES] += 2LL * sv * plan->panel_rmw_rows / m + (passes - 1LL) * (n_tasks * 32 + (long long)plan->st.n_groups * 16);
    } else I[TILESPMV_INFO_X_PANELS] = 1;
    I[TILESPMV_INFO_X_PANEL_MERGE] = plan->st.panel_merge;
    I[TILESPMV_INFO_X_SLICE_PASSES] = plan->st.slice_passes;
    if (plan->st.slice_passes > 0) {
        I[TILESPMV_INFO_X_PANELS] = plan->st.slice_passes;
        I[TILESPMV_INFO_ENTRY_ORDERED] = 0;
        I[TILESPMV_INFO_STREAM_BYTES] += plan->st.slice_passes * 8LL * (n_tasks * 32 + (long long)plan->st.n_groups * 16) + 2LL * sv * std::min<long long>(I[TILESPMV_INFO_SCATTERED_ENTRIES], 8LL * plan->st.slice_passes * plan->panel_rmw_rows / std::max(1, plan->st.x_panels));
    }
    *out = plan;
    return 0;
}

static int plan_from_csr(tilespmv_plan **out, int rowA, int colA, MAT_PTR_TYPE nnzA, const MAT_PTR_TYPE *rowptr, const int *colidx, const MAT_VAL_TYPE *val, unsigned create_flags,
                         const tilespmv_plan_options *opts, bool csr_on_device);

int tilespmv_plan_create_from_csr(tilespmv_plan **out, int rowA, int colA, MAT_PTR_TYPE nnzA, const MAT_PTR_TYPE *rowptr, const int *colidx, const MAT_VAL_TYPE *val, unsigned create_flags,
                                  const tilespmv_plan_options *opts)
{
    return plan_from_csr(out, rowA, colA, nnzA, rowptr, colidx, val, create_flags, opts, false);
}

int tilespmv_plan_create_from_device_csr(tilespmv_plan **out, int rowA, int colA, MAT_PTR_TYPE nnzA, const MAT_PTR_TYPE *d_rowptr, const int *d_colidx, const MAT_VAL_TYPE *d_val, unsigned create_flags,
                                         const tilespmv_plan_options *opts)
{
    return plan_from_csr(out, rowA, colA, nnzA, d_rowptr, d_colidx, d_val, create_flags, opts, true);
}

static int plan_from_csr(tilespmv_plan **out, int rowA, int colA, MAT_PTR_TYPE nnzA, const MAT_PTR_TYPE *rowptr, const int *colidx, const MAT_VAL_TYPE *val, unsigned create_flags,
                         const tilespmv_plan_options *opts, bool csr_on_device)
{
    *out = nullptr;
    const Knobs K = resolve_knobs(opts);
    const bool transpose = (create_flags & TILESPMV_CREATE_TRANSPOSE) != 0;
    if (transpose) std::swap(rowA, colA);
    const int tilen = tiles_of(colA);
    if (K.dry || K.kernel == TILESPMV_KERNEL_DIRECT || tilen > (1 << UNIT_FLAG_SHIFT) || K.coo_mode == TILESPMV_COO_FALLBACK || K.csr_split == 0)
        return -4;
    const double t0 = now_us();
    DevTile *D = nullptr;
    const bool value_map = (create_flags & TILESPMV_CREATE_VALUE_MAP) != 0;
    int rc = 0;
    DevCsrT Tr;
    if (transpose) {
        int ndev = 0;
        if (hipGetDeviceCount(&ndev) != hipSuccess || ndev <= 0) { (void)hipGetLastError(); fprintf(stderr, "tilespmv: no HIP device visible — the device plan builder has no CPU fallback\n"); return -1; }
        rc = devcsr_transpose(&Tr, colA, rowA, rowptr, colidx, val, csr_on_device, !value_map, value_map, value_map && !csr_on_device);
        if (rc == 0) rc = devtile_create(&D, rowA, colA, Tr.rp, Tr.ci, Tr.v, create_flags, false, true, value_map, Tr.src);
        if (rc == 0 && value_map) { (void)hipFree(Tr.src); Tr.src = nullptr; }
    } else
        rc = devtile_create(&D, rowA, colA, rowptr, colidx, val, create_flags, false, csr_on_device, value_map);
    if (rc != 0) return rc;
    const double t1 = now_us();
    Tile_matrix H;
    memset(&H, 0, sizeof(H));
    copy_tile_scalars(H, D->T);
    std::vector<int> h_tile_ptr((size_t)H.tilem + 1, 0), h_tile_col((size_t)std::max(1, H.tilenum), 0);
    std::vector<char> h_fmt((size_t)std::max(1, H.tilenum), 0);
    hipError_t e = hipMemcpy(h_tile_ptr.data(), D->T.tile_ptr, h_tile_ptr.size() * sizeof(int), hipMemcpyDeviceToHost);
    if (e == hipSuccess && H.tilenum > 0) e = hipMemcpy(h_tile_col.data(), D->T.tile_columnidx, (size_t)H.tilenum * sizeof(int), hipMemcpyDeviceToHost);
    if (e == hipSuccess && H.tilenum > 0) e = hipMemcpy(h_fmt.data(), D->T.Format, (size_t)H.tilenum, hipMemcpyDeviceToHost);
    if (e != hipSuccess) { fprintf(stderr, "tilespmv: tile list to the host: %s\n", hipGetErrorString(e)); (void)hipGetLastError(); devtile_destroy(D); return -3; }
    H.tile_ptr = h_tile_ptr.data(); H.tile_columnidx = h_tile_col.data(); H.Format = h_fmt.data();
// ... 250 lines not shown
```

tilespmv_amd/csrc/hip_plan_device.h:

```cpp
#pragma once
#include <vector>

#include "hip_tile_create.h"
#include "plan_tile_ops.h"

namespace tilespmv {

struct DevCounts {
    int csr_form = -1;
    int *tu = nullptr, *tc = nullptr, *td = nullptr;
    int *tp = nullptr;
    int *pool_u = nullptr, *pool_c = nullptr;
    PoolEnt *pool = nullptr;
    void release();
};

struct DevShard { const DevTile *D; int tr0, tr1, t_begin, t_end; bool coo_in_tile, dense_mfma; long long stored0, stored; bool absorb = false, derive = false, verbose = false; };

int dev_fetch_ints(const int *d_array, const long long *idx, int n, int *out);
int dev_count(const DevShard &S, int csr_form, DevCounts *C, hvec<int> &counts3, long long *pool_units = nullptr, long long *pool_lines = nullptr);
int dev_pattern_sample(const DevShard &S, int step, int last_first_tile, int last_rowlen, std::vector<unsigned long long> &patterns);
int dev_emit(const DevShard &S, const DevCounts &C, const hvec<long long> &pu, const hvec<long long> &pc, const hvec<long long> &pd, const std::vector<unsigned char> &row_k,
             const std::vector<unsigned char> &row_split, long long NU, const EmitOut &O);
int dev_fetch_word0(const uint4 *d_udesc, long long NU, hvec<unsigned> &w0);
int dev_pack_desc(const uint4 *d_udesc, const uint2 *d_urow, const uint4 *d_ucol, const int4 *d_map, int ntasks, UDesc *d_packed, URow *d_packed_row, uint4 *d_packed_col);
int dev_all_narrowable(const val_t *d_uval, long long n, bool *all_float, bool *all_half);
int dev_shift_histogram(const UDesc *d_packed, long long NUP, unsigned long long hist[8]);
struct DictRanges { int off[9]; };
int dev_dict_patterns(const UDesc *d_packed, long long NUP, size_t cap, std::vector<uint4> &dict, DictRanges *ranges, bool *over);
int dev_compact_desc(const UDesc *d_packed, long long NUP, const uint4 *d_dict, DictRanges ranges, int cb_bits, unsigned *d_compact);
int dev_pool_dict(const UDesc *d_packed, const URow *d_packed_row, long long NUP, size_t cap, std::vector<uint4> &sorted_patterns, bool *over);
int dev_pool_compact(const UDesc *d_packed, const URow *d_packed_row, long long NUP, const uint4 *d_dict, int ndict, int word_bits, void *d_out);

struct DevLists {
    std::vector<int4> wg;
    long long n_rec = 0, n_chunk = 0, scattered = 0;
    ERec *d_rec = nullptr; unsigned *d_base = nullptr;
    int *d_panel_off = nullptr;
    std::vector<int> panel_off;
    void release();
    ~DevLists() { release(); }
};
int dev_entry_lists(const val_t *d_cval, const int *d_ccol, const unsigned char *d_crow, long long NC, const std::vector<STask> &tasks, int GS, int slab_shift, int dest_bits, bool count_scattered,
                    int x_panels, int panel_shift, DevLists *L);

}
```

tilespmv_amd/csrc/hip_plan_device.hip:

```cpp
#include <cstring>

#include <sys/time.h>

#include <hip/hip_runtime.h>
#include "hip_prims.h"

#include "hip_plan_device.h"

namespace tilespmv {
namespace {

#define PD_TRY(expr)                                                                                                \
    do {                                                                                                            \
        hipError_t e_ = (expr);                                                                                     \
        if (e_ != hipSuccess) {                                                                                     \
            fprintf(stderr, "tilespmv: device plan build: HIP error %d (%s) at %s:%d\n", (int)e_, hipGetErrorString(e_), __FILE__, __LINE__); \
            (void)hipGetLastError();                                                                                \
            return -3;                                                                                              \
        }                                                                                                           \
    } while (0)

typedef unsigned long long u64;
inline unsigned nblk(long long n, int per) { return (unsigned)std::max<long long>(1, (n + per - 1) / per); }

// ... 523 lines not shown
    PD_TRY(hipMemcpy(hn.data(), d_n.p, hn.size() * sizeof(int), hipMemcpyDeviceToHost));
    for (int s = 0; s < nsample; s++) for (int q = 0; q < hn[(size_t)s]; q++) patterns.push_back(hp[(size_t)s * 16 + q]);
    return 0;
}

int dev_emit(const DevShard &S, const DevCounts &C, const hvec<long long> &pu, const hvec<long long> &pc, const hvec<long long> &pd, const std::vector<unsigned char> &row_k,
             const std::vector<unsigned char> &row_split, long long NU, const EmitOut &O)
{
    const DevTile *D = S.D;
    const int nt = S.t_end - S.t_begin, ntr = S.tr1 - S.tr0;
    if (ntr <= 0) return 0;
    auto narrow = [](const hvec<long long> &v) { std::vector<int> o(v.size()); for (size_t i = 0; i < v.size(); i++) o[i] = (int)v[i]; return o; };
    Tmp<int> d_pu, d_pc, d_pd; Tmp<unsigned char> d_rk, d_rs;
    PD_TRY(d_pu.from(narrow(pu))); PD_TRY(d_pc.from(narrow(pc))); PD_TRY(d_pd.from(narrow(pd)));
    PD_TRY(d_rk.from(row_k)); PD_TRY(d_rs.from(row_split));
    if (O.urow && NU > 0) { hipLaunchKernelGGL(k_pd_fill_urow, dim3(nblk(NU, 256)), dim3(256), 0, 0, O.urow, NU); PD_TRY(hipGetLastError()); }
    if (nt > 0) {
        hipLaunchKernelGGL(k_pd_emit_tiles, dim3(nblk(nt, 256)), dim3(256), 0, 0, D->T, D->tile_bi, D->hyb_off, S.t_begin, nt, S.tr0, D->rowA, D->colA, S.coo_in_tile, S.dense_mfma, C.csr_form, S.absorb && C.csr_form < 2, S.derive && C.csr_form < 2, (const int *)C.tu,
                           (const int *)C.tc, (const int *)C.td, (const int *)d_pu.p, (const int *)d_pc.p, (const int *)d_pd.p, (const unsigned char *)d_rk.p, (const unsigned char *)d_rs.p, O);
        PD_TRY(hipGetLastError());
    }
    if (C.csr_form >= 2) {
        hipLaunchKernelGGL(k_pd_emit_pool, dim3(nblk((long long)ntr * 64, 256)), dim3(256), 0, 0, (const int *)D->T.tile_ptr, S.tr0, ntr, S.t_begin, C.csr_form == 3 ? POOL_WIDE_WINDOW : 16u, (const int *)C.tp, (const PoolEnt *)C.pool, (const int *)C.tu, (const int *)C.tc, (const int *)d_pu.p,
                           (const int *)d_pc.p, (const unsigned char *)d_rk.p, O);
        PD_TRY(hipGetLastError());
    }
    PD_TRY(hipDeviceSynchronize());
    return 0;
}

int dev_fetch_word0(const uint4 *d_udesc, long long NU, hvec<unsigned> &w0)
{
    w0.assign((size_t)NU, 0u);
    if (NU <= 0) return 0;
    Tmp<unsigned> d;
    PD_TRY(d.alloc((size_t)NU, false));
    hipLaunchKernelGGL(k_pd_word0, dim3(nblk(NU, 256)), dim3(256), 0, 0, d_udesc, NU, d.p);
    PD_TRY(hipGetLastError());
    PD_TRY(hipMemcpy(w0.data(), d.p, (size_t)NU * sizeof(unsigned), hipMemcpyDeviceToHost));
    return 0;
}

int dev_pack_desc(const uint4 *d_udesc, const uint2 *d_urow, const uint4 *d_ucol, const int4 *d_map, int ntasks, UDesc *d_packed, URow *d_packed_row, uint4 *d_packed_col)
{
    if (ntasks <= 0) return 0;
    hipLaunchKernelGGL(k_pd_pack_desc, dim3((unsigned)std::min(ntasks, 1 << 20)), dim3(256), 0, 0, d_udesc, d_urow, d_ucol, d_map, ntasks, d_packed, d_packed_row, d_packed_col);
    PD_TRY(hipGetLastError());
    PD_TRY(hipDeviceSynchronize());
    return 0;
}

#if !defined(TILESPMV_F32)
__global__ __launch_bounds__(256) void k_pd_not_narrowable(const val_t *__restrict__ v, long long n, unsigned long long *__restrict__ bad)
{
    unsigned nf = 0, nh = 0;
    for (long long i = (long long)blockIdx.x * blockDim.x + threadIdx.x; i < n; i += (long long)gridDim.x * blockDim.x) {
        const val_t a = v[i];
        nf += value_narrowable(a) ? 0u : 1u;
        nh += value_halvable(a) ? 0u : 1u;
    }
    if (nf) atomicAdd(bad, (unsigned long long)nf);
    if (nh) atomicAdd(bad + 1, (unsigned long long)nh);
}
#endif
int dev_all_narrowable(const val_t *d_uval, long long n, bool *all_float, bool *all_half)
{
    *all_float = *all_half = false;
#if !defined(TILESPMV_F32)
    if (n <= 0) { *all_float = *all_half = true; return 0; }
    Tmp<unsigned long long> bad;
    PD_TRY(bad.alloc(2, true));
    hipLaunchKernelGGL(k_pd_not_narrowable, dim3((unsigned)std::min<long long>(nblk(n, 256), 8192)), dim3(256), 0, 0, d_uval, n, bad.p);
    PD_TRY(hipGetLastError());
    unsigned long long h[2] = {1, 1};
    PD_TRY(hipMemcpy(h, bad.p, sizeof(h), hipMemcpyDeviceToHost));
    *all_float = h[0] == 0;
    *all_half = h[1] == 0;
#else
    (void)d_uval; (void)n;
#endif
    return 0;
}

int dev_shift_histogram(const UDesc *d_packed, long long NUP, unsigned long long hist[8])
{
    for (int c = 0; c < 8; c++) hist[c] = 0;
    if (NUP <= 0) return 0;
    Tmp<unsigned long long> h;
    PD_TRY(h.alloc(8, true));
    hipLaunchKernelGGL(k_pd_shift_hist, dim3((unsigned)std::min<long long>(nblk(NUP, 256), 4096)), dim3(256), 0, 0, d_packed, NUP, h.p);
    PD_TRY(hipGetLastError());
    PD_TRY(hipMemcpy(hist, h.p, 8 * sizeof(unsigned long long), hipMemcpyDeviceToHost));
    return 0;
}

int dev_dict_patterns(const UDesc *d_packed, long long NUP, size_t cap, std::vector<uint4> &dict, DictRanges *ranges, bool *over)
{
    dict.clear(); *over = false;
    for (int c = 0; c < 9; c++) ranges->off[c] = 0;
    if (NUP <= 0) return 0;
    Tmp<unsigned long long> hist;
    PD_TRY(hist.alloc(9, true));
    hipLaunchKernelGGL(k_pd_shift_hist, dim3((unsigned)std::min<long long>(nblk(NUP, 256), 4096)), dim3(256), 0, 0, d_packed, NUP, hist.p);
    PD_TRY(hipGetLastError());
    unsigned long long h[9];
    PD_TRY(hipMemcpy(h, hist.p, sizeof(h), hipMemcpyDeviceToHost));
    Tmp<u64> a, b, uniq; Tmp<int> counts, nruns;
    PD_TRY(a.alloc((size_t)NUP, false)); PD_TRY(b.alloc((size_t)NUP, false));
    PD_TRY(uniq.alloc((size_t)NUP, false)); PD_TRY(counts.alloc((size_t)NUP, false)); PD_TRY(nruns.alloc(1, true));
    std::vector<u64> got;
    for (unsigned code = 0; code < 8; code++) {
        ranges->off[code] = (int)dict.size();
        const long long nc = (long long)h[code];
        if (nc == 0) continue;
        PD_TRY(hipMemset(hist.p + 8, 0, sizeof(unsigned long long)));
        hipLaunchKernelGGL(k_pd_patterns, dim3(nblk(NUP, 256)), dim3(256), 0, 0, d_packed, NUP, code, nc == NUP, a.p, hist.p + 8);
        PD_TRY(hipGetLastError());
        u64 *k_cur = a.p, *k_alt = b.p;
        size_t tmp_b = 0; void *tmp = nullptr;
        PD_TRY(prims::sort_keys_u64(nullptr, tmp_b, k_cur, k_alt, (size_t)nc, 0u, 64u, (hipStream_t)0));
        PD_TRY(hipMalloc(&tmp, std::max<size_t>(tmp_b, 16)));
        hipError_t e = prims::sort_keys_u64(tmp, tmp_b, k_cur, k_alt, (size_t)nc, 0u, 64u, (hipStream_t)0);
        (void)hipDeviceSynchronize();
        (void)hipFree(tmp);
        PD_TRY(e);
        PD_TRY(hipMemset(nruns.p, 0, sizeof(int)));
        tmp_b = 0; tmp = nullptr;
        PD_TRY(prims::rle_u64(nullptr, tmp_b, k_cur, 0u, (unsigned)nc, uniq.p, counts.p, nruns.p, (hipStream_t)0));
        PD_TRY(hipMalloc(&tmp, std::max<size_t>(tmp_b, 16)));
        e = prims::rle_u64(tmp, tmp_b, k_cur, 0u, (unsigned)nc, uniq.p, counts.p, nruns.p, (hipStream_t)0);
        int n = 0;
        if (e == hipSuccess) e = hipMemcpy(&n, nruns.p, sizeof(int), hipMemcpyDeviceToHost);
        (void)hipFree(tmp);
        PD_TRY(e);
        if (dict.size() + (size_t)n > cap) { *over = true; dict.clear(); return 0; }
        got.resize((size_t)n);
        PD_TRY(hipMemcpy(got.data(), uniq.p, (size_t)n * sizeof(u64), hipMemcpyDeviceToHost));
        for (u64 k : got) dict.push_back(make_uint4((unsigned)(k >> 32), (unsigned)(k & 0xffffffffull), code << UNIT_SHIFT_SHIFT, 0u));
    }
    ranges->off[8] = (int)dict.size();
    return 0;
}

int dev_pool_dict(const UDesc *d_packed, const URow *d_packed_row, long long NUP, size_t cap, std::vector<uint4> &sorted_patterns, bool *over)
{
    sorted_patterns.clear(); *over = false;
    if (NUP <= 0) return 0;
    Tmp<uint4> table; Tmp<u64> tags; Tmp<int> cnt;
    PD_TRY(table.alloc((size_t)PTABLE, true)); PD_TRY(tags.alloc((size_t)PTABLE, true)); PD_TRY(cnt.alloc(2, true));
    hipLaunchKernelGGL(k_pd_pool_patterns, dim3(nblk(NUP, 256)), dim3(256), 0, 0, d_packed, d_packed_row, NUP, (int)cap, table.p, tags.p, cnt.p);
    PD_TRY(hipGetLastError());
    int h_cnt[2] = {0, 0};
    PD_TRY(hipMemcpy(h_cnt, cnt.p, sizeof(h_cnt), hipMemcpyDeviceToHost));
    if (h_cnt[1] || (size_t)h_cnt[0] > cap) { *over = true; return 0; }
    hipLaunchKernelGGL(k_pd_pool_verify, dim3(nblk(NUP, 256)), dim3(256), 0, 0, d_packed, d_packed_row, NUP, (const uint4 *)table.p, (const u64 *)tags.p, cnt.p);
    PD_TRY(hipGetLastError());
    PD_TRY(hipMemcpy(h_cnt, cnt.p, sizeof(h_cnt), hipMemcpyDeviceToHost));
    if (h_cnt[1]) { *over = true; return 0; }
    std::vector<uint4> ht((size_t)PTABLE); std::vector<u64> hs((size_t)PTABLE);
    PD_TRY(hipMemcpy(ht.data(), table.p, ht.size() * sizeof(uint4), hipMemcpyDeviceToHost));
    PD_TRY(hipMemcpy(hs.data(), tags.p, hs.size() * sizeof(u64), hipMemcpyDeviceToHost));
    for (size_t i = 0; i < ht.size(); i++) if (hs[i] != 0ull) sorted_patterns.push_back(ht[i]);
    std::sort(sorted_patterns.begin(), sorted_patterns.end(), [](const uint4 &a, const uint4 &b) {
        if (a.x != b.x) return a.x < b.x;
        if (a.y != b.y) return a.y < b.y;
        if (a.z != b.z) return a.z < b.z;
// ... 25 lines not shown
```

tilespmv_amd/csrc/hip_plan_internal.h:

```cpp
#pragma once
#include <hip/hip_runtime.h>
#include <sys/time.h>

#include <climits>
#include <cmath>
#include <string>
#include <unordered_map>
#include <unordered_set>

#include "hip_plan.h"
#include "plan_tile_ops.h"

#define HIP_TRY(expr)                                                                                   \
    do {                                                                                                \
        hipError_t e_ = (expr);                                                                         \
        if (e_ != hipSuccess) {                                                                         \
            fprintf(stderr, "tilespmv: HIP error %d (%s) at %s:%d: %s\n", (int)e_, hipGetErrorString(e_), \
                    __FILE__, __LINE__, #expr);                                                         \
            return (int)e_;                                                                             \
        }                                                                                               \
    } while (0)

namespace tilespmv {

inline double now_us()
{
    timeval t;
    gettimeofday(&t, NULL);
    return t.tv_sec * 1e6 + t.tv_usec;
}

inline int env_int(const char *name, int dflt)
{
    const char *e = getenv(name);
    return (e && *e) ? atoi(e) : dflt;
}

struct Knobs {
    int coo_mode, dense_mode, kernel, tilerow_begin, tilerow_end, autotune;
    int entry_mode;
    int entry_ordered;
    int strip_cost;
    int split_above, split_cap, xcd_remap, xcd_chunk, csr_split, fix_inline, coo_cost, coo_heavy_min;
    int coo_piece;
    int strip_even;
    int wg_strips;
    int x_window;
    int x_stride1, x_stride2;
    int lds_pad;
    int y_store;
    int mv_native;
    int mv_xcd_chunk;
    int nt_stream;
    int x_panel_kb;
    int x_panel_merge;
    int x_slice_passes;
    int placement_tries;
    int deterministic;
    int absorb;
    int value_narrow;
    bool value_map;
    int desc_dict;
    bool xcd_from_caller, entry_from_caller, strip_from_caller;
    bool dry;
    const char *autotune_log;
    bool verbose;
    bool placement_force;
    bool encode_check;
    bool encode_on_host;
};

}

using namespace tilespmv;

static inline int slice_trip_records(long long list_records, int groups, int passes)
{
    const double avg = (double)list_records / std::max(1.0, 8.0 * passes * (double)std::max(1, groups));
    return avg * 1.1 <= 1024 ? 4 : avg * 1.1 <= 1536 ? 6 : 8;
}

struct tilespmv_plan {
    DevPlan dev{};
    DevStream st{};
    DevDense dn{};
    int xcd_remap = 2, xcd_chunk = 32;
    val_t *mv_x = nullptr, *mv_y = nullptr;
    int mv_nvec = 0;
    bool mv_by_columns = false;
    int mv_native = -1, mv_xcd_chunk = -1;
    int mv_slab_rows = 0;
    bool pooled = false;
    int entry_mode = 0;
    std::vector<void *> allocs;
    std::vector<std::pair<void *, size_t>> arena_blocks;
    long long info[TILESPMV_INFO_COUNT] = {0};
    int coo_mode = 0, dense_mode = 0, kernel = 0;
    int device = 0;
    int wg_strips = 16;
    int lds_pad_bytes = 0;
    int block_alloc(void **out, size_t bytes, bool quiet = false)
    {
        *out = nullptr;
        hipError_t e = hipMalloc(out, bytes);
        if (e == hipSuccess) e = hipMemset(*out, 0, bytes);
        if (e != hipSuccess) {
            (void)hipGetLastError();
            if (!quiet) fprintf(stderr, "tilespmv: device allocation of %zu MB failed: %s\n", bytes >> 20, hipGetErrorString(e));
            if (*out) (void)hipFree(*out);
            *out = nullptr;
            return -1;
        }
        allocs.push_back(*out);
        return 0;
    }
    void block_free(void *p)
    {
        (void)hipFree(p);
        auto it = std::find(allocs.begin(), allocs.end(), p);
        if (it != allocs.end()) allocs.erase(it);
    }
    static constexpr int VMAP_STREAMS = 5;
    int *vmap = nullptr;
    int vmap_streams = 0;
    const void **vmap_slot[VMAP_STREAMS] = {};
    long long vmap_n[VMAP_STREAMS] = {}, vmap_off[VMAP_STREAMS] = {};
    bool vmap_erec[VMAP_STREAMS] = {};
    size_t arena_used = 0;
    static constexpr size_t arena_block = (size_t)256 << 20;
    char *arena_at = nullptr; size_t arena_left = 0, arena_next = (size_t)1 << 20, size_hint = 0;
    bool dry = false;
    long long list_records = 0;
    bool slice_calibrate = false;
    bool panel_calibrate = false;
    long long panel_rmw_rows = 0;
    unsigned long long digest = 1469598103934665603ull;
    unsigned long long stage_digest[TILESPMV_STAGE_COUNT] = {0};
    std::vector<size_t> uploaded_bytes;
    std::vector<const void **> uploaded_slots;
    int matrix_rows = 0;
    template <class T>
    int reserve(size_t n, const T **out) { return upload<T>(nullptr, n, out); }
// ... 166 lines not shown
```

tilespmv_amd/csrc/hip_plan_stream.hip:

```cpp
#include <array>
#include <mutex>
#include <set>

#include "hip_plan_internal.h"
#include "plan_tile_ops.h"
#include "hip_plan_device.h"

namespace {

struct RowCount { int nunits, ncoo, nheavy, ndense; long long hval, hidx; long long cost; };

inline RowCount count_row(const Tile_matrix *T, int bi, int rowlen, int tilen, int colA, bool coo_in_tile, bool dense_mfma, int csr_form, bool absorb, int coo_cost, const long long *hyb_off, std::vector<PoolEnt> &scratch, long long *pool_stat = nullptr)
{
    RowCount c{0, 0, 0, 0, 0, 0, 0};
    for (int t = T->tile_ptr[bi]; t < T->tile_ptr[bi + 1]; t++) {
        const TileCount k = tile_count(T, t, rowlen, tilen, colA, coo_in_tile, dense_mfma, csr_form, absorb && csr_form < 2, T->tile_ptr[bi], T->tile_ptr[bi + 1]);
        c.nunits += k.nunits; c.ncoo += k.ncoo; c.nheavy += k.nheavy; c.ndense += k.ndense; c.hval += k.hval; c.hidx += k.hidx;
    }
    if (csr_form >= 2) {
        scratch.resize((size_t)std::max<long long>(1, pool_row_capacity(T, bi)));
        int nu, nc, nl;
        pool_row_count(T, bi, rowlen, coo_in_tile, hyb_off, csr_form == 3 ? POOL_WIDE_WINDOW : 16u, scratch.data(), &nu, &nc, &nl);
        c.nunits += nu; c.ncoo += nc;
        if (pool_stat) { pool_stat[0] += nu; pool_stat[1] += nl; }
// ... 3 lines not shown
}


inline void detect_strides(const Tile_matrix *T, int tr0, int tr1, bool csr_split, bool dense_mfma, int *s1, int *s2)
{
    *s1 = *s2 = 0;
    const int ntr = tr1 - tr0;
    if (ntr < 32) return;
    const int step = std::max(1, ntr / 32768);
    std::vector<long long> ds;
    long long sampled = 0;
    for (int bi = tr0; bi < tr1; bi += step) {
        sampled++;
        long long last = LLONG_MIN;
        for (int t = T->tile_ptr[bi]; t < T->tile_ptr[bi + 1]; t++) {
            const int fmt = T->Format[t];
            const bool units = fmt == TILESPMV_FMT_ELL || fmt == TILESPMV_FMT_HYB || fmt == TILESPMV_FMT_DNSCOL || fmt == TILESPMV_FMT_DNSROW ||
                               (fmt == TILESPMV_FMT_DNS && !dense_mfma) || (fmt == TILESPMV_FMT_CSR && csr_split);
            const long long d = (long long)T->tile_columnidx[t] - bi;
            if (units && d >= 2 && d != last) { ds.push_back(d); last = d; }
        }
    }
    std::sort(ds.begin(), ds.end());
    std::vector<long long> dom;
    for (size_t i = 0; i < ds.size();) {
        size_t j = i;
        while (j < ds.size() && ds[j] == ds[i]) j++;
        if ((long long)(j - i) * 4 >= sampled) dom.push_back(ds[i]);
        i = j;
    }
    if (dom.empty() || dom[0] > (1 << 20)) return;
    *s1 = (int)dom[0];
    size_t a = 1;
    while (a < dom.size() && dom[a] <= dom[0] + 1) a++;
    if (a >= dom.size()) return;
    size_t b = a;
    while (b + 1 < dom.size() && dom[b + 1] - dom[b] <= dom[0] + 1) b++;
    const long long mid = dom[(a + b) / 2];
    if (mid % dom[0] == 0 && mid / dom[0] >= 2 && mid < (1ll << 30)) *s2 = (int)mid;
}


struct StreamBuilder {
    tilespmv_plan *plan; const Knobs &K; const Tile_matrix *T; const int rowA, colA, tr0, tr1; const bool coo_in_tile, dense_mfma;
    const std::vector<long long> &hyb_off;
    const long long *hyb_ptr() const { return hyb_off.empty() ? nullptr : hyb_off.data(); }
    DevShard DS{};
    DevCounts dcnt, dcnt_alt;
    uint4 *d_udesc = nullptr, *d_ucol = nullptr; uint2 *d_urow = nullptr; val_t *d_uval = nullptr;
    hvec<unsigned> h_uw0;
    std::vector<FixRow> &fix; int &npartial;
    DevStream &S;
    const DevTile *DT = nullptr;
    int rc = 0;
    bool csr_split = true, pooled = false, wide = false, absorb = false, derive = false; int csr_form = 1, target_in = 0, split_above_in = 0, tilem = 0, tilen = 0, ntr = 0, sv = 0;
    hvec<RowCount> rc_;
    hvec<long long> pu, pc, ph, phv, phi, pd;
    long long NU = 0, NC = 0, NH = 0, NHV = 0, NHI = 0, ND = 0;
    bool fix_inline_on = true, entry_heavy = false, entry_dominated = false, wave_coo = false, coo_ordered = false, brick = false;
    long long total_cost = 0, est_wgs = 0;
    int target = 0, entry_mode = 0, wg_strips = 16, xs1 = 0, xs2 = 0, max_strip_rows = STRIP_MAX_ROWS;
    int panel_shift = 0, x_panels = 1;
    std::vector<STask> tasks;
    std::vector<Task> htasks;
    std::vector<FixRow> ifix, fix_late;
    std::vector<DenseRow> drows;
    std::vector<unsigned char> row_k, row_split;
    int npartial0 = 0;
    std::vector<uint4> h_udesc;
    std::vector<uint2> h_urow;
    std::vector<uint4> h_ucol;
    val_t *h_uval = nullptr, *h_cval = nullptr, *h_hval = nullptr, *h_dval = nullptr;
    unsigned char *h_hidx = nullptr;
    std::vector<int> h_ccol, h_dcb;
    std::vector<unsigned char> h_crow;
    std::vector<uint2> h_hdesc;
    std::vector<uint4> h_udesc_cb;
    long long NUP = 0, n_rec = 0, n_chunk = 0, n_groups = 0, panel_rmw_rows = 0;
    bool pool_dict = false;
    int narrow = 0;
    long long value_bytes() const { return narrow == 2 ? 2 : narrow ? 4 : sv; }
    long long value_group() const { return narrow ? UNIT_GROUP_NARROW : UNIT_GROUP; }
    void choose_value_width();
    int reserve_values()
    {
        if (narrow == 2) return plan->reserve((size_t)NUP * 16, reinterpret_cast<const unsigned short **>(&S.uval));
        if (narrow) return plan->reserve((size_t)NUP * 16, reinterpret_cast<const float **>(&S.uval));
        return plan->reserve((size_t)NUP * 16, &S.uval);
    }
    long long desc_bytes() const { return S.cb_bits > 0 ? 4 : wide ? 28 : pooled ? (pool_dict ? 8 : 20) : 12; }
    std::vector<long long> old_begin;

    StreamBuilder(tilespmv_plan *plan_, const Knobs &K_, const Tile_matrix *T_, int rowA_, int colA_, int tr0_, int tr1_, bool coo_in_tile_, bool dense_mfma_,
                  const std::vector<long long> &hyb_off_, std::vector<FixRow> &fix_, int &npartial_, const DevTile *DT_)
        : plan(plan_), K(K_), T(T_), rowA(rowA_), colA(colA_), tr0(tr0_), tr1(tr1_), coo_in_tile(coo_in_tile_), dense_mfma(dense_mfma_), hyb_off(hyb_off_), fix(fix_), npartial(npartial_), S(plan_->st), DT(DT_) {}
    ~StreamBuilder() { release(); dcnt.release(); dcnt_alt.release(); for (void *q : {(void *)d_udesc, (void *)d_urow, (void *)d_uval, (void *)d_ucol}) if (q) (void)hipFree(q); }
    static void free_later(std::vector<void *> ptrs, size_t bytes_hint)
    {
        ptrs.erase(std::remove(ptrs.begin(), ptrs.end(), (void *)nullptr), ptrs.end());
        if (ptrs.empty()) return;
        if (bytes_hint < ((size_t)64 << 20)) { for (void *q : ptrs) free(q); return; }
        std::thread([ptrs]() { for (void *q : ptrs) free(q); }).detach();
    }
    void release()
    {
        free_later({h_uval, h_cval, h_hval, h_hidx, h_dval}, (size_t)(NU * 16 + NC + NHV + ND * 256) * sizeof(val_t));
        h_uval = h_cval = h_hval = h_dval = nullptr; h_hidx = nullptr;
    }

    struct Hash {
        unsigned long long h = 1469598103934665603ull;
        void bytes(const void *p, size_t len) { const unsigned char *b = (const unsigned char *)p; for (size_t i = 0; i < len; i++) { h ^= b[i]; h *= 1099511628211ull; } }
        template <class V, class A> void vec(const std::vector<V, A> &v) { arr(v.data(), v.size()); }
        template <class V> void arr(const V *p, size_t n) { const unsigned long long cnt = n; bytes(&cnt, 8); if (n) bytes(p, n * sizeof(V)); }
        void num(long long v) { bytes(&v, 8); }
    };
    bool hashing() const { return plan->dry; }
    void stage_done(int stage, const Hash &h) { plan->stage_digest[stage] = h.h; }

    void count();
    void choose();
    void cut();
    void emit();
    void order();
    void encode();
    void encode_device();
    void entries();
    void finish(long long &n_tasks, long long &model_bytes);
};

void StreamBuilder::count()
{
    target_in = K.strip_cost; split_above_in = K.split_above;
    tilem = T->tilem; tilen = T->tilen; ntr = std::max(0, tr1 - tr0); sv = (int)sizeof(val_t);
    csr_form = K.csr_split < 0 ? 1 : std::min(K.csr_split, 3);
    absorb = K.absorb != 0 && coo_in_tile;
    derive = absorb && K.absorb != 2;
    const int t_begin = T->tile_ptr[tr0], t_end = T->tile_ptr[tr1];
    if (DT) {
        DS = DevShard{DT, tr0, tr1, t_begin, t_end, coo_in_tile, dense_mfma, 0, 0, absorb, derive, K.verbose};
        const long long idx[2] = {t_begin, t_end}; int v[2] = {0, 0};
        if (dev_fetch_ints(DT->T.blknnz, idx, 2, v) != 0) { rc = -3; return; }
        DS.stored0 = v[0]; DS.stored = (long long)v[1] - v[0];
    }
    long long pool_units_of[4] = {0, 0, 0, 0}, pool_lines_of[4] = {0, 0, 0, 0};
    auto count_all = [&](int form, hvec<RowCount> &out) {
        out.assign((size_t)ntr, RowCount{0, 0, 0, 0, 0, 0, 0});
        if (DT) {
            hvec<int> k3;
            DevCounts &C = form == csr_form ? dcnt : dcnt_alt;
            if (dev_count(DS, form, &C, k3, &pool_units_of[form], &pool_lines_of[form]) != 0) { rc = -3; return; }
            parallel_chunks(ntr, 1 << 16, [&](int64_t b, int64_t e, int) {
                for (int64_t i = b; i < e; i++) {
                    RowCount c{k3[3 * (size_t)i], k3[3 * (size_t)i + 1], 0, k3[3 * (size_t)i + 2], 0, 0, 0};
                    c.cost = 16LL * c.nunits + (long long)K.coo_cost * c.ncoo + 64LL * c.ndense + 8;
                    out[(size_t)i] = c;
                }
            });
            return;
        }
        std::mutex stat_mutex;
        parallel_chunks(ntr, 1024, [&](int64_t b, int64_t e, int) {
            std::vector<PoolEnt> scratch;
            long long st[2] = {0, 0};
            for (int64_t i = b; i < e; i++) out[i] = count_row(T, tr0 + (int)i, tile_rowlen(tr0 + (int)i, tilem, rowA), tilen, colA, coo_in_tile, dense_mfma, form, absorb, K.coo_cost, hyb_ptr(), scratch, st);
            std::lock_guard<std::mutex> lk(stat_mutex);
// ... 438 lines not shown
            }
        });
        all_float = not_float.load() == 0;
        all_half = not_half.load() == 0;
    }
    narrow = may_half && all_half ? 2 : may_float && all_float ? 1 : 0;
    if (K.verbose) fprintf(stderr, "tilespmv: unit values: %s\n", narrow == 2 ? "every one is a half: stored in 2 bytes" : narrow ? "every one is a float: stored in 4 bytes" : "8 bytes (not all of them survive the narrowing the knob and the size rule allow)");
}

void StreamBuilder::encode_device()
{
    const long long G = value_group();
    auto padded = [&](long long n) { return (n + G - 1) / G * G; };
    std::vector<int4> pair_map(tasks.size());
    old_begin.assign(tasks.size(), 0);
    long long at = 0;
    for (size_t i = 0; i < tasks.size(); i++) {
        STask &k = tasks[i];
        const long long ub = k.unit_begin, n = k.unit_end - ub, nb = at;
        old_begin[i] = ub;
        at += padded(n);
        pair_map[i] = make_int4((int)ub, (int)nb, (int)n, 0);
        if (n > 0) { k.unit_begin = (int)nb; k.unit_end = (int)(nb + n); }
    }
    const double t0 = now_us();
    const long long up0 = plan->info[TILESPMV_INFO_UPLOAD_US];
    S.udict = nullptr; S.cb_bits = 0; S.urow = nullptr; S.ucol = nullptr; S.pooled = pooled ? 1 : 0; S.pdict = nullptr; pool_dict = false;
    void *d_map = nullptr; UDesc *d_packed = nullptr; URow *d_prow = nullptr;
    auto fail = [&](const char *what, hipError_t e) { fprintf(stderr, "tilespmv: device plan build: %s: %s\n", what, hipGetErrorString(e)); (void)hipGetLastError(); rc = -3; };
    hipError_t e = hipMalloc(&d_map, std::max<size_t>(pair_map.size(), 1) * sizeof(int4));
    if (e == hipSuccess && !pair_map.empty()) e = hipMemcpy(d_map, pair_map.data(), pair_map.size() * sizeof(int4), hipMemcpyHostToDevice);
    if (e == hipSuccess) e = hipMalloc((void **)&d_packed, std::max<long long>(NUP, 1) * sizeof(UDesc) + 256);
    if (e == hipSuccess) e = hipMemsetAsync(d_packed, 0, std::max<long long>(NUP, 1) * sizeof(UDesc) + 256, 0);
    if (e != hipSuccess) fail("scratch for the packed descriptors", e);
    if (wide) rc |= plan->reserve((size_t)NUP, &S.ucol);
    if (pooled && !wide && e == hipSuccess) {
        e = hipMalloc((void **)&d_prow, std::max<long long>(NUP, 1) * sizeof(URow) + 256);
        if (e == hipSuccess) e = hipMemsetAsync(d_prow, 0, std::max<long long>(NUP, 1) * sizeof(URow) + 256, 0);
        if (e != hipSuccess) fail("scratch for the packed row nibbles", e);
    }
    if (rc == 0 && dev_pack_desc(d_udesc, d_urow, d_ucol, (const int4 *)d_map, (int)pair_map.size(), d_packed, d_prow, const_cast<uint4 *>(S.ucol)) != 0) rc = -3;
    if (rc == 0 && pooled && !wide && K.desc_dict != 0 && NUP > 0) {
        std::vector<uint4> pats;
        bool over = false;
        if (dev_pool_dict(d_packed, d_prow, NUP, (size_t)1 << DICT_MAX_BITS, pats, &over) != 0) rc = -3;
        else if (!over) {
            rc |= plan->upload(pats.data(), pats.size(), &S.pdict);
            const int bb = pool_word_base_bits((int)pats.size());
            const bool word = K.desc_dict != 2 && POOL_STRIP_ROWS <= 4 && bb >= 4 && (long long)T->tilen * 16 <= (1ll << bb);
            if (word) rc |= plan->reserve((size_t)NUP, reinterpret_cast<const unsigned **>(&S.udesc));
            else rc |= plan->reserve((size_t)NUP, reinterpret_cast<const uint2 **>(&S.udesc));
            if (rc == 0 && dev_pool_compact(d_packed, d_prow, NUP, S.pdict, (int)pats.size(), word ? bb : 0, const_cast<UDesc *>(S.udesc)) != 0) rc = -3;
            pool_dict = true;
            if (word) S.cb_bits = bb;
        }
    }
    if (rc == 0 && pooled && !wide && !pool_dict) {
        rc |= plan->reserve((size_t)NUP, &S.urow);
        if (rc == 0 && NUP > 0 && (e = hipMemcpy(const_cast<URow *>(S.urow), d_prow, (size_t)NUP * sizeof(URow), hipMemcpyDeviceToDevice)) != hipSuccess) fail("row nibble copy", e);
    }
    const bool dict_pays = K.desc_dict > 0 ? true : 8LL * NUP * 50 >= NUP * (12 + 16LL * sv) + NC * (sv + 4LL);
    if (rc == 0 && K.desc_dict != 0 && dict_pays && !pooled && NUP > 0) {
        const int cb_bits = std::max(1, 32 - __builtin_clz((unsigned)std::max(1, T->tilen - 1)));
        const int pid_bits = std::min(DICT_MAX_BITS, 27 - cb_bits);
        if (pid_bits >= 1) {
            std::vector<uint4> dict;
            DictRanges ranges;
            bool over = false;
            if (dev_dict_patterns(d_packed, NUP, (size_t)1 << pid_bits, dict, &ranges, &over) != 0) rc = -3;
            else if (!over) {
                rc |= plan->upload(dict.data(), dict.size(), &S.udict);
                rc |= plan->reserve((size_t)NUP, reinterpret_cast<const unsigned **>(&S.udesc));
                if (rc == 0 && dev_compact_desc(d_packed, NUP, S.udict, ranges, cb_bits, reinterpret_cast<unsigned *>(const_cast<UDesc *>(S.udesc))) != 0) rc = -3;
                S.cb_bits = cb_bits;
            }
        }
    }
    if (rc == 0 && S.cb_bits == 0 && !pool_dict) {
        rc |= plan->reserve((size_t)NUP, &S.udesc);
        if (rc == 0 && NUP > 0 && (e = hipMemcpy(const_cast<UDesc *>(S.udesc), d_packed, (size_t)NUP * sizeof(UDesc), hipMemcpyDeviceToDevice)) != hipSuccess) fail("descriptor copy", e);
    }
    plan->info[TILESPMV_INFO_DESC_BYTES] = desc_bytes();
    if (rc == 0 && !pooled) { unsigned long long hist[8]; if (dev_shift_histogram(d_packed, NUP, hist) != 0) rc = -3; else plan->info[TILESPMV_INFO_DERIVED_UNITS] = (long long)hist[UNIT_DERIVED_CODE]; }
    rc |= reserve_values();
    if (rc == 0) {
        e = launch_pair_values(d_uval, const_cast<val_t *>(S.uval), (const int4 *)d_map, (int)pair_map.size(), narrow);
        if (e == hipSuccess) e = hipDeviceSynchronize();
        if (e != hipSuccess) fail("value pass", e);
    }
    for (void *q : {(void *)d_map, (void *)d_packed, (void *)d_prow, (void *)d_udesc, (void *)d_urow, (void *)d_uval, (void *)d_ucol}) if (q) (void)hipFree(q);
    d_udesc = nullptr; d_urow = nullptr; d_uval = nullptr; d_ucol = nullptr;
    S.udesc_cb = S.udesc;
    plan->info[TILESPMV_INFO_UPLOAD_US] = up0 + (long long)(now_us() - t0);
}

void StreamBuilder::encode()
{
    const unsigned long long d0 = plan->digest;
    choose_value_width();
    if (rc) return;
    S.uval_narrow = narrow;
    if (narrow == 2) plan->size_hint -= std::min(plan->size_hint, (size_t)(NU * 16 * (sv - value_bytes())));
    const long long G = value_group();
    auto padded = [&](long long n) { return (n + G - 1) / G * G; };
    NUP = 0;
    for (const STask &k : tasks) NUP += padded(k.unit_end - k.unit_begin);
    if (NUP > INT32_MAX) {
        fprintf(stderr, "tilespmv: shard too large for 32-bit unit ids\n");
        rc = -2;
        return;
    }
    if (DT) { encode_device(); return; }
    {
        std::vector<UDesc> packed((size_t)NUP, UDesc{0u, 0u, 0u});
        std::vector<URow> packed_row(pooled && !wide ? (size_t)NUP : 0, URow{0u, 0u});
        std::vector<uint4> packed_col(wide ? (size_t)NUP : 0, make_uint4(0u, 0u, 0u, 0u));
        const bool encode_check = !plan->dry && K.encode_check;
        const bool on_device = !plan->dry && NUP > 0 && !K.encode_on_host;
        val_t *paired = (on_device && !encode_check) || narrow ? nullptr : zalloc<val_t>((size_t)NUP * 16);
        float *paired_n = (on_device && !encode_check) || narrow != 1 ? nullptr : zalloc<float>((size_t)NUP * 16);
        unsigned short *paired_h = (on_device && !encode_check) || narrow != 2 ? nullptr : zalloc<unsigned short>((size_t)NUP * 16);
        std::vector<int4> pair_map(on_device ? tasks.size() : 0);
        std::vector<long long> new_begin(tasks.size());
        old_begin.assign(tasks.size(), 0);
        for (size_t i = 0; i < tasks.size(); i++) old_begin[i] = tasks[i].unit_begin;
        long long at = 0;
        for (size_t i = 0; i < tasks.size(); i++) { new_begin[i] = at; at += padded(tasks[i].unit_end - tasks[i].unit_begin); }
        parallel_chunks((int64_t)tasks.size(), 512, [&](int64_t b, int64_t e, int) {
            for (int64_t i = b; i < e; i++) {
                STask &k = tasks[(size_t)i];
                const long long ub = k.unit_begin, n = k.unit_end - ub, nb = new_begin[(size_t)i];
                for (long long j = 0; j < n; j++) {
                    const uint4 d = h_udesc[(size_t)(ub + j)];
                    packed[(size_t)(nb + j)] = UDesc{d.x, d.y, d.w};
                    if (pooled && !wide) packed_row[(size_t)(nb + j)] = URow{h_urow[(size_t)(ub + j)].x, h_urow[(size_t)(ub + j)].y};
                    if (wide) packed_col[(size_t)(nb + j)] = h_ucol[(size_t)(ub + j)];
                    if (paired) {
                        const val_t *src = h_uval + (ub + j) * 16;
                        val_t *dst = paired + (nb + j / G * G) * 16 + (j % G);
                        for (int r = 0; r < 16; r++) dst[G * r] = src[r];
                    }
                    if (paired_n) {
                        const val_t *src = h_uval + (ub + j) * 16;
                        float *dst = paired_n + (nb + j / G * G) * 16 + (j % G);
                        for (int r = 0; r < 16; r++) dst[G * r] = (float)src[r];
                    }
                    if (paired_h) {
                        const val_t *src = h_uval + (ub + j) * 16;
                        unsigned short *dst = paired_h + (nb + j / G * G) * 16 + (j % G);
                        for (int r = 0; r < 16; r++) dst[G * r] = value_half_bits((double)src[r]);
                    }
                }
                if (on_device) pair_map[(size_t)i] = make_int4((int)ub, (int)nb, (int)n, 0);
                if (n > 0) { k.unit_begin = (int)nb; k.unit_end = (int)(nb + n); }
            }
        });
        S.udict = nullptr; S.cb_bits = 0;
        std::vector<uint4> dict;
        std::vector<unsigned> compact;
        const bool dict_pays = K.desc_dict > 0 ? true : 8LL * NUP * 50 >= NUP * (12 + 16LL * sv) + NC * (sv + 4LL);
        if (K.desc_dict != 0 && dict_pays && !pooled && NUP > 0) {
            const int cb_bits = std::max(1, 32 - __builtin_clz((unsigned)std::max(1, T->tilen - 1)));
            const int pid_bits = std::min(DICT_MAX_BITS, 27 - cb_bits);
            if (pid_bits >= 1) {
                const size_t cap = (size_t)1 << pid_bits;
                typedef std::pair<unsigned, unsigned long long> Pat;
                std::vector<std::array<std::unordered_set<unsigned long long>, 8>> local((size_t)host_threads());
                std::atomic<int> over(0);
                parallel_chunks((int64_t)NUP, 1 << 16, [&](int64_t b, int64_t e, int th) {
                    if (over.load(std::memory_order_relaxed)) return;
                    auto &L = local[(size_t)th];
                    size_t have = 0;
                    for (auto &q : L) have += q.size();
                    for (int64_t u = b; u < e; u++) {
                        if (L[packed[(size_t)u].w0 >> UNIT_SHIFT_SHIFT].insert(((unsigned long long)packed[(size_t)u].n0 << 32) | packed[(size_t)u].n1).second) have++;
                        if (have > cap) { over.store(1); return; }
                    }
                });
                std::vector<Pat> all;
                if (!over.load()) {
                    for (auto &L : local) for (unsigned sc = 0; sc < 8; sc++) for (unsigned long long k : L[sc]) all.push_back(Pat(sc, k));
                    std::sort(all.begin(), all.end());
                    all.erase(std::unique(all.begin(), all.end()), all.end());
                }
                if (!over.load() && all.size() <= cap) {
                    dict.resize(all.size());
                    for (size_t i = 0; i < all.size(); i++) dict[i] = make_uint4((unsigned)(all[i].second >> 32), (unsigned)(all[i].second & 0xffffffffull), all[i].first << UNIT_SHIFT_SHIFT, 0u);
                    compact.resize((size_t)NUP);
                    const unsigned cbmask = (1u << cb_bits) - 1u;
                    parallel_chunks((int64_t)NUP, 1 << 16, [&](int64_t b, int64_t e, int) {
                        for (int64_t u = b; u < e; u++) {
                            const UDesc &d = packed[(size_t)u];
                            const Pat key(d.w0 >> UNIT_SHIFT_SHIFT, ((unsigned long long)d.n0 << 32) | d.n1);
                            const unsigned pid = (unsigned)(std::lower_bound(all.begin(), all.end(), key) - all.begin());
                            compact[(size_t)u] = (d.w0 & cbmask) | (pid << cb_bits) | ((d.w0 >> UNIT_FLAG_SHIFT) << 27);
                        }
                    });
                    S.cb_bits = cb_bits;
                }
            }
        }
        S.pdict = nullptr; pool_dict = false;
        std::vector<uint4> pdict;
        std::vector<uint2> compact2;
        std::vector<unsigned> compact1;
        if (pooled && !wide && K.desc_dict != 0 && NUP > 0) {
            typedef std::array<unsigned, 4> Pat;
            const size_t cap = (size_t)1 << DICT_MAX_BITS;
            std::vector<std::set<Pat>> local((size_t)host_threads());
            std::atomic<int> over(0);
            parallel_chunks((int64_t)NUP, 1 << 16, [&](int64_t b, int64_t e, int th) {
                if (over.load(std::memory_order_relaxed)) return;
                std::set<Pat> &L = local[(size_t)th];
                Pat last{{~0u, ~0u, ~0u, ~0u}};
                for (int64_t u = b; u < e; u++) {
                    const Pat q{{packed[(size_t)u].n0, packed[(size_t)u].n1, packed_row[(size_t)u].r0, packed_row[(size_t)u].r1}};
                    if (q == last) continue;
                    last = q;
                    L.insert(q);
                    if (L.size() > cap) { over.store(1); return; }
                }
            });
            std::vector<Pat> all;
            if (!over.load()) {
                for (auto &L : local) all.insert(all.end(), L.begin(), L.end());
                std::sort(all.begin(), all.end());
                all.erase(std::unique(all.begin(), all.end()), all.end());
            }
            if (!over.load() && all.size() <= cap) {
                pdict.resize(all.size());
                for (size_t i = 0; i < all.size(); i++) pdict[i] = make_uint4(all[i][0], all[i][1], all[i][2], all[i][3]);
                compact2.resize((size_t)NUP);
                parallel_chunks((int64_t)NUP, 1 << 16, [&](int64_t b, int64_t e, int) {
                    for (int64_t u = b; u < e; u++) {
                        const Pat q{{packed[(size_t)u].n0, packed[(size_t)u].n1, packed_row[(size_t)u].r0, packed_row[(size_t)u].r1}};
                        compact2[(size_t)u] = make_uint2(packed[(size_t)u].w0, (unsigned)(std::lower_bound(all.begin(), all.end(), q) - all.begin()));
                    }
                });
                pool_dict = true;
                const int bb = pool_word_base_bits((int)all.size());
                if (K.desc_dict != 2 && POOL_STRIP_ROWS <= 4 && bb >= 4 && (long long)T->tilen * 16 <= (1ll << bb)) {
                    compact1.resize((size_t)NUP);
                    parallel_chunks((int64_t)NUP, 1 << 16, [&](int64_t b, int64_t e, int) {
                        for (int64_t u = b; u < e; u++) {
                            const uint2 c = compact2[(size_t)u];
                            compact1[(size_t)u] = (c.x & POOL_BASE_MASK) | (c.y << bb) | ((c.x >> POOL_KR_SHIFT) << POOL_WORD_KR_SHIFT);
                        }
                    });
                    S.cb_bits = bb;
                }
            }
        }
        S.urow = nullptr; S.ucol = nullptr; S.pooled = pooled ? 1 : 0;
        if (pool_dict) {
            if (S.cb_bits > 0) rc |= plan->upload(compact1.data(), compact1.size(), reinterpret_cast<const unsigned **>(&S.udesc));
            else rc |= plan->upload(compact2.data(), compact2.size(), reinterpret_cast<const uint2 **>(&S.udesc));
            rc |= plan->upload(pdict.data(), pdict.size(), &S.pdict);
        } else if (S.cb_bits > 0) {
            rc |= plan->upload(compact.data(), compact.size(), reinterpret_cast<const unsigned **>(&S.udesc));
            rc |= plan->upload(dict.data(), dict.size(), &S.udict);
        } else rc |= plan->upload(packed.data(), (size_t)NUP, &S.udesc);
        plan->info[TILESPMV_INFO_DESC_BYTES] = desc_bytes();
        if (!pooled) { long long nder = 0; for (long long u = 0; u < NUP; u++) nder += (packed[(size_t)u].w0 >> UNIT_SHIFT_SHIFT) == UNIT_DERIVED_CODE; plan->info[TILESPMV_INFO_DERIVED_UNITS] = nder; }
        if (pooled && !wide && !pool_dict) rc |= plan->upload(packed_row.data(), (size_t)NUP, &S.urow);
        if (wide) rc |= plan->upload(packed_col.data(), (size_t)NUP, &S.ucol);
        if (on_device) {
            const double t0 = now_us();
            void *d_src = nullptr, *d_map = nullptr;
            const size_t src_b = (size_t)NU * 16 * sizeof(val_t), map_b = pair_map.size() * sizeof(int4);
            rc |= reserve_values();
            hipError_t e = hipMalloc(&d_src, std::max<size_t>(src_b, 16));
            if (e == hipSuccess) e = hipMalloc(&d_map, std::max<size_t>(map_b, 16));
            if (e == hipSuccess) e = hipMemcpy(d_src, h_uval, src_b, hipMemcpyHostToDevice);
            if (e == hipSuccess) e = hipMemcpy(d_map, pair_map.data(), map_b, hipMemcpyHostToDevice);
            if (e == hipSuccess && rc == 0) e = launch_pair_values((const val_t *)d_src, const_cast<val_t *>(S.uval), (const int4 *)d_map, (int)pair_map.size(), narrow);
            if (e == hipSuccess) e = hipDeviceSynchronize();
            if (e == hipSuccess && encode_check) {
                std::vector<unsigned char> back((size_t)NUP * 16 * (size_t)value_bytes());
                e = hipMemcpy(back.data(), S.uval, back.size(), hipMemcpyDeviceToHost);
                if (e == hipSuccess && memcmp(back.data(), narrow == 2 ? (const void *)paired_h : narrow ? (const void *)paired_n : (const void *)paired, back.size()) != 0) { fprintf(stderr, "tilespmv: internal error: the device's value stream differs from the host's\n"); rc = -6; }
                else if (e == hipSuccess && K.verbose) fprintf(stderr, "tilespmv: encode check: %lld units, device value stream == host value stream\n", NUP);
            }
            if (d_src) (void)hipFree(d_src);
            if (d_map) (void)hipFree(d_map);
            if (e != hipSuccess) { fprintf(stderr, "tilespmv: value pass on the device failed: %s\n", hipGetErrorString(e)); (void)hipGetLastError(); rc = -3; }
            plan->info[TILESPMV_INFO_UPLOAD_US] += (long long)(now_us() - t0);
        } else if (narrow == 2) rc |= plan->upload(paired_h, (size_t)NUP * 16, reinterpret_cast<const unsigned short **>(&S.uval));
        else if (narrow) rc |= plan->upload(paired_n, (size_t)NUP * 16, reinterpret_cast<const float **>(&S.uval));
        else rc |= plan->upload(paired, (size_t)NUP * 16, &S.uval);
        free_later({paired, paired_n, paired_h, h_uval}, (size_t)NUP * 16 * sizeof(val_t));
        h_uval = nullptr;
        S.udesc_cb = S.udesc;
    }
    if (hashing()) { Hash h; h.num((long long)(plan->digest ^ d0)); h.num(NUP); h.num(S.cb_bits); h.num(S.pooled); if (pool_dict) h.num(8); stage_done(TILESPMV_STAGE_ENCODE, h); }
}

void StreamBuilder::entries()
{
    const unsigned long long d0 = plan->digest;
    S.wg_coo = nullptr; S.grec = nullptr; S.gbase = nullptr; S.dest_bits = 11;
    n_rec = 0; n_chunk = 0; n_groups = 0;
    if (entry_mode != 0) {
        const size_t GS = entry_mode == 2 ? (size_t)wg_strips : 4;
        const int slab_shift = pooled ? (POOL_STRIP_ROWS > 4 ? 7 : 6) : 7;
        const int dest_bits = entry_mode == 2 ? (wg_strips == 32 ? 12 : 4 + slab_shift) : 9;
        S.dest_bits = dest_bits;
        const size_t nwg = (tasks.size() + GS - 1) / GS;
        const size_t NP = (size_t)x_panels;
        std::vector<std::vector<ERec>> grp_rec(nwg);
        std::vector<std::vector<unsigned>> grp_base(nwg);
        std::vector<int> h_panel_off(NP > 1 ? nwg * (NP + 1) : 0, 0);
        std::atomic<int> bad(0);
        std::atomic<long long> scattered(0);
        DevLists dlists;
        if (DT) {
            if (dev_entry_lists(S.cval, S.ccol, S.crow, NC, tasks, (int)GS, slab_shift, dest_bits, entry_mode == 2, x_panels, panel_shift, &dlists) != 0) { rc = -3; return; }
            scattered.store(dlists.scattered);
            if (NP > 1) h_panel_off = dlists.panel_off;
        }
        parallel_chunks(DT ? 0 : (int64_t)nwg, 64, [&](int64_t b, int64_t e, int) {
            std::vector<std::pair<unsigned long long, unsigned>> key;
            std::vector<int> src;
            std::vector<PEnt> ents;
            for (int64_t w = b; w < e; w++) {
                key.clear(); src.clear();
                long long own_lo = LLONG_MAX, own_hi = LLONG_MIN;
                for (size_t t = GS * (size_t)w; t < std::min(tasks.size(), GS * (size_t)w + GS); t++) {
                    own_lo = std::min<long long>(own_lo, 16LL * tasks[t].row); own_hi = std::max<long long>(own_hi, 16LL * (tasks[t].row + std::max(1, tasks[t].nrows)));
                    for (int q = tasks[t].coo_begin; q < tasks[t].coo_end; q++) {
                        key.push_back({((unsigned long long)(unsigned)h_ccol[(size_t)q] << 32) | (unsigned long long)key.size(),
                                       (unsigned)((t & (GS - 1)) << slab_shift) | (unsigned)h_crow[(size_t)q]});
                        src.push_back(q);
                    }
                }
                std::sort(key.begin(), key.end());
                ents.resize(key.size());
                for (size_t i = 0; i < key.size(); i++) {
                    const int q = src[(size_t)(key[i].first & 0xFFFFFFFFull)];
                    ents[i] = PEnt{(unsigned)h_ccol[(size_t)q], key[i].second, h_cval[q]};
                }
                if (entry_mode == 2) {
                    long long far = 0;
                    for (const PEnt &en : ents) far += !((long long)en.col >= own_lo - 2048 && (long long)en.col < own_hi + 2048);
                    scattered.fetch_add(far, std::memory_order_relaxed);
                }
                if (!pack_list(ents, dest_bits, grp_rec[(size_t)w], grp_base[(size_t)w], plan->dry)) bad++;
// ... 171 lines not shown
```

tilespmv_amd/csrc/hip_units_kernel.h:

```cpp
#pragma once
#include <hip/hip_runtime.h>

#include <type_traits>

#include "hip_plan.h"

namespace tilespmv {

typedef double lacc_t;

template <int CTRL>
__device__ __forceinline__ double dpp_mov(double v)
{
    int lo = __double2loint(v), hi = __double2hiint(v);
    lo = __builtin_amdgcn_update_dpp(0, lo, CTRL, 0xF, 0xF, false);
    hi = __builtin_amdgcn_update_dpp(0, hi, CTRL, 0xF, 0xF, false);
    return __hiloint2double(hi, lo);
}
template <int CTRL>
__device__ __forceinline__ float dpp_mov(float v)
{
    return __int_as_float(__builtin_amdgcn_update_dpp(0, __float_as_int(v), CTRL, 0xF, 0xF, false));
}
template <class T>
// ... 98 lines not shown
    return __uint_as_float(r.v);
#else
    return __hiloint2double((int)r.hi, (int)r.lo);
#endif
}

template <int CT>
__device__ __forceinline__ void wave_entry_trips(const DevStream &S, const val_t *__restrict__ x, lacc_t *swave, int lane, int gb, int ge, int chunk0, int cfirst)
{
    const int db = S.dest_bits;
    const unsigned dmask = (1u << db) - 1u;
    const int clast = chunk0 + ((ge - 1 - gb) >> 6);
    for (int e0 = gb + 64 * cfirst; e0 < ge; e0 += 64 * CT) {
        ERec rr[CT]; unsigned cb[CT]; val_t xx[CT];
#pragma unroll
        for (int q = 0; q < CT; q++) {
            rr[q] = S.grec[min(e0 + 64 * q + lane, ge - 1)];
            cb[q] = S.gbase[__builtin_amdgcn_readfirstlane(min(chunk0 + ((e0 - gb) >> 6) + q, clast))];
        }
#pragma unroll
        for (int q = 0; q < CT; q++) xx[q] = x[(size_t)(cb[q] + (rr[q].w >> db))];
#pragma unroll
        for (int q = 0; q < CT; q++)
            if (e0 + 64 * q + lane < ge) atomicAdd(&swave[rr[q].w & dmask], (lacc_t)(erec_val(rr[q]) * xx[q]));
    }
}

#ifndef WG_TRIP_PIPE
#define WG_TRIP_PIPE 0
#endif

template <int CT, int NT, bool NTL>
__device__ __forceinline__ void wg_entry_trips(const ERec *__restrict__ rec, const unsigned *__restrict__ base, int chunk0, int db, bool ordered,
                                               const val_t *__restrict__ x, lacc_t *sy, int tid, int gb, int ge, int gs = -1)
{
    if (gs < 0) gs = gb;
    const int e_first = gb + ((gs - gb) & ~63);
    const unsigned dmask = (1u << db) - 1u;
    const int wave = tid >> 6;
    const int clast = chunk0 + ((ge - 1 - gb) >> 6);
    ERec rr[CT]; unsigned cb[CT];
    auto load_trip = [&](int e0, ERec (&r)[CT], unsigned (&c)[CT]) {
#pragma unroll
        for (int q = 0; q < CT; q++) {
            if constexpr (NTL) {
                const unsigned *pw = reinterpret_cast<const unsigned *>(&rec[min(e0 + NT * q + tid, ge - 1)]);
                unsigned *rw = reinterpret_cast<unsigned *>(&r[q]);
#pragma unroll
                for (int z = 0; z < (int)(sizeof(ERec) / 4); z++) rw[z] = __builtin_nontemporal_load(pw + z);
            } else r[q] = rec[min(e0 + NT * q + tid, ge - 1)];
            c[q] = base[__builtin_amdgcn_readfirstlane(min(chunk0 + ((e0 - gb) >> 6) + (NT / 64) * q + wave, clast))];
        }
    };
    if (e_first < ge) load_trip(e_first, rr, cb);
    for (int e0 = e_first; e0 < ge; e0 += NT * CT) {
        val_t xx[CT];
        if (!WG_TRIP_PIPE && e0 > e_first) load_trip(e0, rr, cb);
#pragma unroll
        for (int q = 0; q < CT; q++) xx[q] = x[(size_t)(cb[q] + (rr[q].w >> db))];
        ERec rn[CT]; unsigned cn[CT];
        if (WG_TRIP_PIPE) load_trip(min(e0 + NT * CT, gb + (ge - 1 - gb) / (NT * CT) * (NT * CT)), rn, cn);
        if (ordered) {
            for (int w = 0; w < NT / 64; w++) {
                if (wave == w) {
#pragma unroll
                    for (int q = 0; q < CT; q++)
                        if (e0 + NT * q + tid < ge && e0 + NT * q + tid >= gs) atomicAdd(&sy[rr[q].w & dmask], (lacc_t)(erec_val(rr[q]) * xx[q]));
                }
                __syncthreads();
            }
        } else {
#pragma unroll
            for (int q = 0; q < CT; q++)
                if (e0 + NT * q + tid < ge && e0 + NT * q + tid >= gs) atomicAdd(&sy[rr[q].w & dmask], (lacc_t)(erec_val(rr[q]) * xx[q]));
        }
        if (WG_TRIP_PIPE) {
#pragma unroll
            for (int q = 0; q < CT; q++) { rr[q] = rn[q]; cb[q] = cn[q]; }
        }
    }
}

extern __shared__ __attribute__((aligned(16))) unsigned char s_dyn[];
#if defined(UNITS_KERNEL) != defined(UNITS_NARROW_FORM)
#error "hip_units_kernel.h: define UNITS_KERNEL and UNITS_NARROW_FORM together (or neither: k_units, floats)"
#endif
#ifndef UNITS_KERNEL
#define UNITS_KERNEL k_units
#define UNITS_NARROW_FORM 1
#endif
template <int UB, int ECOO, int GPB, bool CD, bool NTS, bool POOL = false, bool WIDE = false, bool NARROW = false>
__global__ __launch_bounds__(16 * GPB, ECOO == 1 ? 4 : ECOO == 2 ? (POOL ? POOL_ECOO2_MIN_WAVES : NARROW && UNITS_NARROW_FORM == 2 ? UNITS_MIN_WAVES : ECOO2_MIN_WAVES) : POOL ? (WIDE ? 6 : POOL_MIN_WAVES) : UNITS_MIN_WAVES) void UNITS_KERNEL(DevStream S, int rowA, int colA, int xcd_chunk, val_t *__restrict__ partial,
                                               const val_t *__restrict__ x, val_t *__restrict__ y)
{
    constexpr int VFORM = NARROW ? UNITS_NARROW_FORM : 0;
    static_assert(VFORM >= 0 && VFORM <= 2, "UNITS_NARROW_FORM: 1 or 2");
    static_assert(!NARROW || (sizeof(val_t) == 8 && !POOL && ECOO != 1 && GPB == 16 && NTS), "narrow values: fp64 classic plans, entry mode 0 / 2, 16 strips, nontemporal streams");
    constexpr int G = NARROW ? UNIT_GROUP_NARROW : UNIT_GROUP;
    static_assert(DCHUNK % UB == 0 && UB % G == 0, "a batch never straddles a descriptor chunk and is whole value groups");
    static_assert(GPB == 16 || (GPB == 32 && ECOO == 2) || (GPB == 8 && ECOO != 2 && !NTS), "512-thread workgroups exist for the workgroup entry mode only, 128-thread ones for small grids without it");
    static_assert(!(NTS && ECOO == 1), "nontemporal streams: large plans only (entry mode 1 = small grids)");
    static_assert(!POOL || GPB == 16 || GPB == 8, "pooled plans: 256-thread workgroups (128 on small grids)");
    static_assert(!WIDE || (POOL && !CD), "wide windows: pooled plans, 12-B descriptors + 16 B of column offsets");
    constexpr int GROUPS_PER_BLOCK = GPB;
    constexpr int SROWS = POOL ? POOL_STRIP_ROWS : STRIP_MAX_ROWS;
    constexpr bool NT = NTS;
#ifndef TILESPMV_NT_DESC
#define TILESPMV_NT_DESC 0
#endif
#ifndef TILESPMV_NT_COO0
#define TILESPMV_NT_COO0 0
#endif
    constexpr bool NT_DESC = NTS && TILESPMV_NT_DESC, NT_COO0 = NTS && TILESPMV_NT_COO0;
    constexpr bool PCOPY = POOL && sizeof(val_t) == 4;
    constexpr int SLAB = GROUPS_PER_BLOCK * SROWS * 16;
    __shared__ lacc_t s_yall[SLAB + (PCOPY ? SLAB + 16 : 0)];
    lacc_t (*s_y)[SROWS][16] = reinterpret_cast<lacc_t (*)[SROWS][16]>(&s_yall[0]);
    lacc_t *s_y1 = &s_yall[PCOPY ? SLAB + 16 : 0];
    __shared__ uint4 s_d[GROUPS_PER_BLOCK][DCHUNK];
    __shared__ uint2 s_r[POOL && !WIDE ? GROUPS_PER_BLOCK : 1][POOL && !WIDE ? DCHUNK : 1];
    __shared__ uint4 s_c[WIDE ? GROUPS_PER_BLOCK : 1][WIDE ? DCHUNK : 1];
    const int tid = threadIdx.x, r = tid & 15, g = tid >> 4;
    unsigned bid = blockIdx.x;
    if (xcd_chunk > 0) {
        const unsigned C = (unsigned)xcd_chunk, W = 8u * C, win = bid / W, off = bid % W, k = off & 7u;
        if ((win + 1) * W <= gridDim.x) bid = win * W + k * C + (off >> 3);
    }
    const long long task_id = (long long)bid * GROUPS_PER_BLOCK + g;
    const bool have = task_id < S.ntasks;
    constexpr bool WCOO = ECOO == 1;
    if (ECOO == 1) { if ((long long)bid * GROUPS_PER_BLOCK + (g & ~3) >= S.ntasks) return; }
    else if (ECOO == 0 && !have) return;
    int4 t0 = make_int4(0, 0, 0, 0), t1 = make_int4(0, -1, 0, 0);
    if (have) {
        t0 = reinterpret_cast<const int4 *>(S.task)[task_id * 2];
        t1 = reinterpret_cast<const int4 *>(S.task)[task_id * 2 + 1];
    }
    const int unit_begin = t0.x, unit_end = t0.y, coo_begin = t0.z, coo_end = t0.w;
    const int row0 = t1.x, part = t1.y, nrows = t1.w;
    const unsigned nounit = (unsigned)t1.z;
    const bool side = POOL || coo_end > coo_begin;
    if constexpr (POOL) {
        for (int k = 0; k < nrows; k++) { s_y[g][k][r] = 0; if constexpr (PCOPY) s_y1[(g * SROWS + k) * 16 + r] = 0; }
        wave_lds_fence();
    }
    typedef std::conditional_t<VFORM == 2, _Float16, std::conditional_t<VFORM == 1, float, val_t>> sval_t;
    typedef sval_t grp_t __attribute__((ext_vector_type(G)));
    const grp_t *__restrict__ ugrp = reinterpret_cast<const grp_t *>(S.uval) + r;
    const int last = unit_end - 1;
    const int last_grp = unit_begin + (unit_end - 1 - unit_begin) / G * G;
    const bool have_units = unit_begin < unit_end;
    const long long xlast = (long long)colA - 1;
    const int xlast32 = colA - 1;
    const int ncoo = coo_end - coo_begin;
    uint4 dcur = make_uint4(0u, 0u, 0u, 0u), dnext = dcur;
    uint2 rcur = make_uint2(0u, 0u), rnext = rcur;
    const uint2 *__restrict__ urw = reinterpret_cast<const uint2 *>(S.urow);
    uint4 ccur = make_uint4(0u, 0u, 0u, 0u), cnext = ccur;
    unsigned wnn = 0;
    const unsigned *__restrict__ udw = reinterpret_cast<const unsigned *>(S.udesc);
    uint2 wnn2 = make_uint2(0u, 0u);
    val_t v[UB];
    auto unit_prologue = [&]() {
        if (have_units) {
            if constexpr (CD && POOL) {
                const uint2 a = pool_desc(S, min(unit_begin + r, last)), b = pool_desc(S, min(unit_begin + DCHUNK + r, last));
                dcur.x = a.x; dcur.y = a.y; dnext.x = b.x; dnext.y = b.y;
            } else if constexpr (CD) {
                dcur.x = stream_load<NT_DESC>(udw + min(unit_begin + r, last));
                dnext.x = stream_load<NT_DESC>(udw + min(unit_begin + DCHUNK + r, last));
            } else {
                dcur = load_udesc_raw(S.udesc, min(unit_begin + r, last));
                dnext = load_udesc_raw(S.udesc, min(unit_begin + DCHUNK + r, last));
                if constexpr (WIDE) { ccur = S.ucol[min(unit_begin + r, last)]; cnext = S.ucol[min(unit_begin + DCHUNK + r, last)]; }
                else if constexpr (POOL) { rcur = urw[min(unit_begin + r, last)]; rnext = urw[min(unit_begin + DCHUNK + r, last)]; }
            }
#pragma unroll
            for (int k = 0; k < UB; k += G) {
                const grp_t pv = stream_load<NT>(ugrp + (long long)min(unit_begin + k, last_grp) * (16 / G));
#pragma unroll
                for (int q = 0; q < G; q++) v[k + q] = pv[q];
            }
        }
    };

    const uint2 *sd = reinterpret_cast<const uint2 *>(&s_d[g][0]) + (r >> 3);
    uint2 d[UB];
    unsigned rw[UB];
    val_t xv[UB];
    const unsigned *sr = reinterpret_cast<const unsigned *>(&s_r[POOL && !WIDE ? g : 0][0]) + (r >> 3);
    const unsigned char *sc = reinterpret_cast<const unsigned char *>(&s_c[WIDE ? g : 0][0]) + r;
    auto park_first = [&]() {
        if constexpr (CD && POOL) {
            const uint4 p0 = S.pdict[dcur.y], p1 = S.pdict[dnext.y];
            wnn2 = pool_desc(S, min(unit_begin + 2 * DCHUNK + r, last));
            s_d[g][r] = make_uint4(dcur.x, p0.x, dcur.x, p0.y); s_r[g][r] = make_uint2(p0.z, p0.w);
            dnext = make_uint4(dnext.x, p1.x, 0u, p1.y); rnext = make_uint2(p1.z, p1.w);
        } else if constexpr (CD) {
            const uint4 p0 = udict_of(S, dcur.x), p1 = udict_of(S, dnext.x);
            wnn = stream_load<NT_DESC>(udw + min(unit_begin + 2 * DCHUNK + r, last));
            dnext.y = p1.x; dnext.z = p1.z; dnext.w = p1.y;
            s_d[g][r] = udesc_expand(S, dcur.x, p0);
        } else s_d[g][r] = udesc_park_form(dcur);
        if constexpr (WIDE) s_c[g][r] = ccur;
        else if constexpr (POOL && !CD) s_r[g][r] = rcur;
    };
    auto fetch_batch = [&](int j0) {
#pragma unroll
        for (int k = 0; k < UB; k++) d[k] = sd[2 * (j0 + k)];
        if constexpr (WIDE) {
#pragma unroll
            for (int k = 0; k < UB; k++) rw[k] = d[k].y;
#pragma unroll
            for (int k = 0; k < UB; k++) {
                if constexpr (UNIT_X32) xv[k] = x[x_index32((int)(d[k].x & POOL_BASE_MASK), sc[16 * (j0 + k)], xlast32)];
                else xv[k] = x[min((long long)(d[k].x & POOL_BASE_MASK) + (long long)sc[16 * (j0 + k)], xlast)];
            }
            return;
        }
        if constexpr (POOL) {
#pragma unroll
            for (int k = 0; k < UB; k++) rw[k] = sr[2 * (j0 + k)];
#pragma unroll
            for (int k = 0; k < UB; k++) {
                if constexpr (UNIT_X32) xv[k] = x[x_index32((int)(d[k].x & POOL_BASE_MASK), (d[k].y >> (28 - 4 * (r & 7))) & 15u, xlast32)];
                else xv[k] = x[min((long long)(d[k].x & POOL_BASE_MASK) + (long long)((d[k].y >> (28 - 4 * (r & 7))) & 15u), xlast)];
            }
            return;
        }
#pragma unroll
        for (int k = 0; k < UB; k++) {
            const unsigned fl = d[k].x >> 24;
            const unsigned nib = (fl & UNIT_ROWUNIT) ? (unsigned)r : (d[k].y >> (28 - 4 * (r & 7))) & 15u;
            if ((d[k].x >> UNIT_SHIFT_SHIFT) == UNIT_DERIVED_CODE && r != 15) xv[k] = 0;
            else if constexpr (UNIT_X32) xv[k] = x[x_index32(unit_x_base32(d[k].x), nib, xlast32)];
            else xv[k] = x[min(unit_x_base(d[k].x) + nib, xlast)];
        }
    };

    if constexpr (ECOO == 2) {
        const int4 wr = S.wg_coo[bid];
        if (wr.y > wr.x) {
            if (side) for (int k = 0; k < nrows; k++) s_y[g][k][r] = 0;
            __syncthreads();
        } else if ((S.panel_merge > 0 || S.slice_passes > 0) && side) {
            for (int k = 0; k < nrows; k++) s_y[g][k][r] = 0;
            wave_lds_fence();
        }
        constexpr bool LATE_PROLOGUE = VFORM == 2;
        if constexpr (!LATE_PROLOGUE) unit_prologue();
        if (wr.y > wr.x) {
            int ge = wr.y;
            if (GPB == 16 && S.panel_merge > 0) ge = S.panel_off[(size_t)bid * (size_t)(S.x_panels + 1) + (size_t)min(S.x_panels, S.panel_merge)];
            if (GPB == 16 && S.slice_passes > 0) ge = wr.x;
            wg_entry_trips<WCOO_HEAVY_CT, 16 * GPB, NTS>(S.grec, S.gbase, wr.z, S.dest_bits, S.coo_ordered != 0, x, &s_y[0][0][0], tid, wr.x, ge);
            __syncthreads();
        }
        if constexpr (LATE_PROLOGUE) unit_prologue();
    } else if constexpr (WCOO) {
        constexpr int CT = 6;
        const int lane = tid & 63;
        const int4 wr = S.wg_coo[(long long)bid * (GROUPS_PER_BLOCK / 4) + (g >> 2)];
        const int tot = wr.y - wr.x;
        lacc_t *swave = &s_y[g & ~3][0][0];
        unit_prologue();
        ERec rr[CT]; unsigned cbase[CT]; val_t xx[CT];
        const int db = S.dest_bits;
        if (tot > 0) {
            if (side) for (int k = 0; k < nrows; k++) s_y[g][k][r] = 0;
            const int clast = wr.z + ((tot - 1) >> 6);
#pragma unroll
            for (int q = 0; q < CT; q++) {
                rr[q] = S.grec[min(wr.x + 64 * q + lane, wr.y - 1)];
                cbase[q] = S.gbase[__builtin_amdgcn_readfirstlane(min(wr.z + q, clast))];
            }
        }
        if (have_units) {
            park_first();
            wave_lds_fence();
            fetch_batch(0);
        } else if (tot > 0) wave_lds_fence();
        if (tot > 0) {
            const unsigned dmask = (1u << db) - 1u;
#pragma unroll
            for (int q = 0; q < CT; q++) xx[q] = x[(size_t)(cbase[q] + (rr[q].w >> db))];
#pragma unroll
            for (int q = 0; q < CT; q++)
                if (wr.x + 64 * q + lane < wr.y) atomicAdd(&swave[rr[q].w & dmask], (lacc_t)(erec_val(rr[q]) * xx[q]));
            if (tot > 64 * CT) wave_entry_trips<CT>(S, x, swave, lane, wr.x, wr.y, wr.z, CT);
            wave_lds_fence();
        }
    } else {
    constexpr int CT = 6;
    const bool coo_heavy = ncoo > S.coo_heavy_min;
    if (side) {
        for (int k = 0; k < nrows; k++) s_y[g][k][r] = 0;
        wave_lds_fence();
    }
    if (coo_heavy) {
        for (int e0 = coo_begin; e0 < coo_end; e0 += 16 * CT) {
            unsigned rb[CT]; int cc[CT]; val_t cv[CT], xx[CT];
#pragma unroll
            for (int q = 0; q < CT; q++) {
                const int e = min(e0 + 16 * q + r, coo_end - 1);
                rb[q] = S.crow[e]; cc[q] = S.ccol[e]; cv[q] = S.cval[e];
            }
#pragma unroll
            for (int q = 0; q < CT; q++) xx[q] = x[cc[q]];
#pragma unroll
            for (int q = 0; q < CT; q++)
                if (e0 + 16 * q + r < coo_end) atomicAdd(&s_y[g][rb[q] >> 4][rb[q] & 15u], (lacc_t)(cv[q] * xx[q]));
        }
        wave_lds_fence();
    }
    unsigned rb0 = 0; int cc0 = 0; val_t cv0 = 0;
    const bool coo0 = side && !coo_heavy && (coo_begin + r < coo_end);
    if (coo0) { rb0 = stream_load<NT_COO0>(S.crow + coo_begin + r); cc0 = stream_load<NT_COO0>(S.ccol + coo_begin + r); cv0 = stream_load<NT_COO0>(S.cval + coo_begin + r); }
    unit_prologue();
    if (side && !coo_heavy) {
        if (coo0) atomicAdd(&s_y[g][rb0 >> 4][rb0 & 15u], (lacc_t)(cv0 * x[cc0]));
        for (int e0 = coo_begin + 16; e0 < coo_end; e0 += 64) {
            unsigned rb[4]; int cc[4]; val_t cv[4], xx[4];
#pragma unroll
            for (int q = 0; q < 4; q++) {
                const int e = min(e0 + 16 * q + r, coo_end - 1);
                rb[q] = S.crow[e]; cc[q] = S.ccol[e]; cv[q] = S.cval[e];
            }
#pragma unroll
            for (int q = 0; q < 4; q++) xx[q] = x[cc[q]];
#pragma unroll
            for (int q = 0; q < 4; q++)
                if (e0 + 16 * q + r < coo_end) atomicAdd(&s_y[g][rb[q] >> 4][rb[q] & 15u], (lacc_t)(cv[q] * xx[q]));
        }
        wave_lds_fence();
    }
    }

    val_t acc = 0;
    auto retire = [&](val_t prod, unsigned flags, unsigned word1) {
        if constexpr (POOL) {
            const unsigned dest = ((flags >> (POOL_KR_SHIFT - 24)) & 7u) * 16u + ((word1 >> (28 - 4 * (r & 7))) & 15u);
            if constexpr (PCOPY) atomicAdd(((r & 1) ? s_y1 : &s_y[0][0][0]) + g * (SROWS * 16) + dest, (lacc_t)prod);
            else atomicAdd(&s_y[g][0][0] + dest, (lacc_t)prod);
            return;
        }
        if (flags & UNIT_ROWUNIT) {
            prod = strip_allreduce(prod);
            if (r != (int)(word1 & 15u)) prod = 0;
        }
        acc += prod;
        if (flags & UNIT_EOR) {
            const int kr = (int)((flags >> UNIT_ROW_SHIFT) & 7u);
            if constexpr (sizeof(val_t) == sizeof(lacc_t)) {
                lacc_t out = acc;
                if (side) out += s_y[g][kr][r];
                s_y[g][kr][r] = out;
            } else {
                val_t out = acc;
                if (side) out = (val_t)((lacc_t)acc + s_y[g][kr][r]);
                reinterpret_cast<val_t *>(&s_y[g][kr][0])[r] = out;
            }
            acc = 0;
        }
    };
    if (have_units) {
        if (ECOO != 1) {
            park_first();
            wave_lds_fence();
        }
        int chunk_end = unit_begin + DCHUNK;
        val_t xprev = 0;
        for (int u = unit_begin; u < unit_end; u += UB) {
            if (u == chunk_end) {
                wave_lds_fence();
                if constexpr (CD && POOL) { s_d[g][r] = make_uint4(dnext.x, dnext.y, dnext.x, dnext.w); s_r[g][r] = rnext; }
                else if constexpr (CD) s_d[g][r] = udesc_expand(S, dnext.x, make_uint4(dnext.y, dnext.w, dnext.z, 0u));
                else s_d[g][r] = udesc_park_form(dnext);
                if constexpr (WIDE) { s_c[g][r] = cnext; cnext = S.ucol[min(chunk_end + DCHUNK + r, last)]; }
                else if constexpr (POOL && !CD) { s_r[g][r] = rnext; rnext = urw[min(chunk_end + DCHUNK + r, last)]; }
                wave_lds_fence();
                chunk_end += DCHUNK;
                if constexpr (CD && POOL) {
                    const uint4 p = S.pdict[wnn2.y];
                    dnext = make_uint4(wnn2.x, p.x, 0u, p.y); rnext = make_uint2(p.z, p.w);
                    wnn2 = pool_desc(S, min(chunk_end + DCHUNK + r, last));
                } else if constexpr (CD) {
                    const uint4 p = udict_of(S, wnn);
                    dnext = make_uint4(wnn, p.x, p.z, p.y);
                    wnn = stream_load<NT_DESC>(udw + min(chunk_end + DCHUNK + r, last));
                } else dnext = load_udesc_raw(S.udesc, min(chunk_end + r, last));
            }
            if (!(ECOO == 1 && u == unit_begin)) fetch_batch(u - (chunk_end - DCHUNK));
            sval_t vn[UB];
#pragma unroll
            for (int k = 0; k < UB; k += G) {
                const grp_t *pa = ugrp + (long long)min(u + UB + k, last_grp) * (16 / G);
                if constexpr (UNIT_TAIL_HOT) pa = (u + UB + k <= last_grp) ? pa : reinterpret_cast<const grp_t *>(S.uval);
                const grp_t pv = stream_load<NT>(pa);
#pragma unroll
                for (int q = 0; q < G; q++) vn[k + q] = pv[q];
            }
#pragma unroll
            for (int k = 0; k < UB; k++)
            {
                if constexpr (POOL) {
                    retire((u + k < unit_end) ? v[k] * xv[k] : (val_t)0, d[k].x >> 24, rw[k]);
                } else {
                    const val_t xu = unit_x_use(xv[k], xprev, d[k].x, r);
                    xprev = xu;
                    if (u + k < unit_end) retire(v[k] * xu, d[k].x >> 24, d[k].y);
                }
            }
#pragma unroll
            for (int k = 0; k < UB; k++) v[k] = vn[k];
        }
    }
    if constexpr (POOL) {
        wave_lds_fence();
        if constexpr (PCOPY) {
            for (int k = 0; k < nrows; k++) s_y[g][k][r] += s_y1[(g * SROWS + k) * 16 + r];
            wave_lds_fence();
        }
    }
    if (part >= 0) {
        val_t out = acc;
        if (side) out = (val_t)((lacc_t)acc + s_y[g][0][r]);
        if (S.ifix_count == nullptr || nounit == 0xFFFFFFFFu) {
            partial[(long long)part * 16 + r] = out;
        } else {
            __hip_atomic_store(&partial[(long long)part * 16 + r], out, __ATOMIC_RELAXED, __HIP_MEMORY_SCOPE_AGENT);
            __builtin_amdgcn_fence(__ATOMIC_RELEASE, "wavefront");
            asm volatile("s_waitcnt vmcnt(0)" ::: "memory");
            const FixRow f = S.ifix[nounit];
            unsigned prev = 0;
            if (r == 0) prev = __hip_atomic_fetch_add(&S.ifix_count[nounit], 1u, __ATOMIC_RELAXED, __HIP_MEMORY_SCOPE_AGENT);
            prev = (unsigned)__shfl((int)prev, tid & 48, 64);
            __builtin_amdgcn_fence(__ATOMIC_ACQUIRE, "wavefront");
            if (prev == (unsigned)f.count - 1u) {
                val_t sum = 0;
                for (int k0 = 0; k0 < f.count; k0 += 8) {
                    val_t sv[8];
#pragma unroll
                    for (int j = 0; j < 8; j++)
                        sv[j] = __hip_atomic_load(&partial[(long long)(f.first + min(k0 + j, f.count - 1)) * 16 + r], __ATOMIC_RELAXED, __HIP_MEMORY_SCOPE_AGENT);
#pragma unroll
                    for (int j = 0; j < 8; j++) if (k0 + j < f.count) sum += sv[j];
                }
                const long long yi = (long long)f.row * 16 + r;
                if (yi < rowA) y[yi] = sum;
                if (r == 0) __hip_atomic_store(&S.ifix_count[nounit], 0u, __ATOMIC_RELAXED, __HIP_MEMORY_SCOPE_AGENT);
            }
        }
    } else {
        if constexpr (POOL) {
// ... 48 lines not shown
```

Baseline: 1586 GFLOP/s.

## Add lean units kernel specialized for plans without row-units or derived units

Adds a plan-time scan that records whether any unit carries the row-unit flag or the derived-shift code. When neither or only one is present, a new template instantiation of the units kernel compiles out the row-unit allreduce and, optionally, the derived-x handling. Its main loop is split into full batches and a single tail batch, and the value prefetch pointer is advanced incrementally. This is meant to cut per-unit branches, register pressure and tail checks, at the cost of another kernel variant, an extra device counting pass during plan build, and a new default-on knob.

Result: faster. 1604 GFLOP/s (median of 6 runs) (+1.2%).

```diff
diff --git a/include/tilespmv.h b/include/tilespmv.h
--- a/include/tilespmv.h
+++ b/include/tilespmv.h
@@ -193,6 +193,7 @@
     int deterministic;
     int absorb;
     int value_narrow;
+    int unit_lean;
     int reserved[1];
 } tilespmv_plan_options;
 void tilespmv_plan_options_init(tilespmv_plan_options *opts);
@@ -269,7 +270,7 @@
     TILESPMV_INFO_DESC_BYTES = 20,
     TILESPMV_INFO_NT_STREAM = 21,
     TILESPMV_INFO_UNIT_VALUE_BYTES = 22,
-    TILESPMV_INFO_RETIRED_23 = 23,
+    TILESPMV_INFO_UNIT_LEAN = 23,
     TILESPMV_INFO_PLACEMENT_TRIES = 24,
     TILESPMV_INFO_RETIRED_25 = 25,
     TILESPMV_INFO_X_PANELS = 26,
diff --git a/tilespmv_amd/_lib.py b/tilespmv_amd/_lib.py
--- a/tilespmv_amd/_lib.py
+++ b/tilespmv_amd/_lib.py
@@ -13,13 +13,13 @@
 
 INFO_NAMES = ["device_bytes", "stream_bytes", "nnz", "rows", "tiles", "coo_mode", "dense_mode", "kernel",
               "num_tasks", "num_split_rows", "fallback_nnz", "build_us", "upload_us", "entry_mode", "entry_ordered", "strip_cost",
-              "wg_strips", "list_entries", "derived_units", "brick_order", "desc_bytes", "nt_stream", "unit_value_bytes", "retired_23", "placement_tries", "retired_25", "x_panels", "x_panel_merge", "scattered_entries", "x_slice_passes", "csr_form", "timed_choices_us", "device_build", "tile_create_us",
+              "wg_strips", "list_entries", "derived_units", "brick_order", "desc_bytes", "nt_stream", "unit_value_bytes", "unit_lean", "placement_tries", "retired_25", "x_panels", "x_panel_merge", "scattered_entries", "x_slice_passes", "csr_form", "timed_choices_us", "device_build", "tile_create_us",
               "value_map_bytes"]
 
 
 KNOB_DEFAULT = -1
 KNOB_NAMES = ["entry_mode", "entry_ordered", "strip_cost", "split_above", "split_cap", "xcd_remap", "xcd_chunk", "csr_split", "fix_inline",
-              "coo_cost", "coo_heavy_min", "coo_piece", "strip_even", "wg_strips", "x_window", "x_stride1", "x_stride2", "mv_native", "mv_xcd_chunk", "lds_pad", "y_store", "desc_dict", "nt_stream", "x_panel_kb", "x_panel_merge", "placement_tries", "x_slice_passes", "deterministic", "absorb", "value_narrow"]
+              "coo_cost", "coo_heavy_min", "coo_piece", "strip_even", "wg_strips", "x_window", "x_stride1", "x_stride2", "mv_native", "mv_xcd_chunk", "lds_pad", "y_store", "desc_dict", "nt_stream", "x_panel_kb", "x_panel_merge", "placement_tries", "x_slice_passes", "deterministic", "absorb", "value_narrow", "unit_lean"]
 
 
 class PlanOptions(C.Structure):
diff --git a/tilespmv_amd/csrc/hip_kernels.hip b/tilespmv_amd/csrc/hip_kernels.hip
--- a/tilespmv_amd/csrc/hip_kernels.hip
+++ b/tilespmv_amd/csrc/hip_kernels.hip
@@ -1152,6 +1152,10 @@
 #define TSPMV_FORM(W, B) TSPMV_FORM_(W, B, TSPMV_NTS)
 #define TSPMV_FORM_SMALL(W, B) TSPMV_FORM_(W, B, TSPMV_PLAIN)
         const bool small_grid = entry_mode != 2 && !S.nt_stream && (S.ntasks + 15) / 16 < SMALL_GRID_WORKGROUPS;
+        if (const int lean = unit_lean_form(S, entry_mode, wg_strips)) {
+            const hipError_t el = launch_units_lean(P, S, lean, entry_mode, wg_strips, lds_pad_bytes, xc, x, y, st);
+            if (el != hipSuccess) return el;
+        } else
 #if !defined(TILESPMV_F32)
         if (S.uval_narrow == 2) {
             const hipError_t eh = launch_units_half(P, S, entry_mode, wg_strips, lds_pad_bytes, xc, x, y, st);
diff --git a/tilespmv_amd/csrc/hip_kernels_lean.hip b/tilespmv_amd/csrc/hip_kernels_lean.hip
--- /dev/null
+++ b/tilespmv_amd/csrc/hip_kernels_lean.hip
@@ -0,0 +1,32 @@
+#include <hip/hip_runtime.h>
+
+#include "hip_plan.h"
+#include "hip_plan_internal.h"
+
+#define UNITS_KERNEL k_units_lean
+#define UNITS_LEAN 1
+#include "hip_units_kernel.h"
+
+namespace tilespmv {
+
+hipError_t launch_units_lean(const DevPlan &P, const DevStream &S, int form, int entry_mode, int wg_strips, int lds_pad_bytes, int xcd_chunk, const val_t *x, val_t *y, hipStream_t st)
+{
+    if (form != unit_lean_form(S, entry_mode, wg_strips) || form < 1) return hipErrorInvalidValue;
+#define TSPMV_KL(W, CD, VF, DV) hipLaunchKernelGGL((k_units_lean<TILESPMV_UB, W, 16, CD, true, VF, DV>), dim3((unsigned)((S.ntasks + 15) / 16)), dim3(256), (size_t)lds_pad_bytes, st, S, P.rowA, P.colA, xcd_chunk, P.partial, x, y)
+#define TSPMV_KL_DV(W, CD, VF) do { if (form == 1) TSPMV_KL(W, CD, VF, true); else TSPMV_KL(W, CD, VF, false); } while (0)
+#define TSPMV_KL_CD(W, VF) do { if (S.cb_bits > 0) TSPMV_KL_DV(W, true, VF); else TSPMV_KL_DV(W, false, VF); } while (0)
+#define TSPMV_KL_W(VF) do { if (entry_mode == 2) TSPMV_KL_CD(2, VF); else TSPMV_KL_CD(0, VF); } while (0)
+#if !defined(TILESPMV_F32)
+    if (S.uval_narrow == 2) TSPMV_KL_W(2);
+    else if (S.uval_narrow == 1) TSPMV_KL_W(1);
+    else
+#endif
+    TSPMV_KL_W(0);
+#undef TSPMV_KL_W
+#undef TSPMV_KL_CD
+#undef TSPMV_KL_DV
+#undef TSPMV_KL
+    return hipGetLastError();
+}
+
+}
diff --git a/tilespmv_amd/csrc/hip_plan.h b/tilespmv_amd/csrc/hip_plan.h
--- a/tilespmv_amd/csrc/hip_plan.h
+++ b/tilespmv_amd/csrc/hip_plan.h
@@ -127,7 +127,16 @@
     const UDesc *udesc_cb;
     const FixRow *ifix;
     unsigned *ifix_count;
+    int unit_facts;
+    int unit_lean;
 };
+constexpr int UNIT_FACT_NO_ROWUNIT = 1, UNIT_FACT_NO_DERIVED = 2;
+inline int unit_lean_form(const DevStream &S, int entry_mode, int wg_strips)
+{
+    if (!S.unit_lean || S.ntasks <= 0 || S.pooled || !S.nt_stream || !(entry_mode == 0 || entry_mode == 2) || wg_strips != 16) return 0;
+    if (!(S.unit_facts & UNIT_FACT_NO_ROWUNIT)) return 0;
+    return (S.unit_facts & UNIT_FACT_NO_DERIVED) ? 2 : 1;
+}
 
 struct DenseRow { int row, tile_begin, tile_end, partial; };
 __host__ __device__ constexpr int dense_slot(int r, int c)
@@ -157,5 +166,6 @@
 }
 
 hipError_t launch_units_half(const DevPlan &P, const DevStream &S, int entry_mode, int wg_strips, int lds_pad_bytes, int xcd_chunk, const val_t *x, val_t *y, hipStream_t st);
+hipError_t launch_units_lean(const DevPlan &P, const DevStream &S, int form, int entry_mode, int wg_strips, int lds_pad_bytes, int xcd_chunk, const val_t *x, val_t *y, hipStream_t st);
 
 }
diff --git a/tilespmv_amd/csrc/hip_plan.hip b/tilespmv_amd/csrc/hip_plan.hip
--- a/tilespmv_amd/csrc/hip_plan.hip
+++ b/tilespmv_amd/csrc/hip_plan.hip
@@ -59,6 +59,8 @@
     k.x_slice_passes = pick(o.x_slice_passes, "TILESPMV_X_SLICE_PASSES", -1);
     k.absorb = pick(o.absorb, "TILESPMV_ABSORB", -1); if (k.absorb < 0 || k.absorb > 2) k.absorb = 1;
     k.value_narrow = pick(o.value_narrow, "TILESPMV_VALUE_NARROW", -1);
+    static const int unit_lean_env = env_int("TILESPMV_UNIT_LEAN", 1);
+    k.unit_lean = (o.unit_lean != TILESPMV_KNOB_DEFAULT ? o.unit_lean : unit_lean_env) != 0 ? 1 : 0;
     k.deterministic = pick(o.deterministic, "TILESPMV_DETERMINISTIC", 0) > 0 ? 1 : 0;
     if (k.deterministic) {
         if (k.placement_tries < 0) k.placement_tries = 1;
@@ -235,7 +237,7 @@
         TSPMV_F(entry_mode) TSPMV_F(entry_ordered) TSPMV_F(strip_cost) TSPMV_F(split_above) TSPMV_F(split_cap) TSPMV_F(xcd_remap) TSPMV_F(xcd_chunk)
         TSPMV_F(csr_split) TSPMV_F(fix_inline) TSPMV_F(coo_cost) TSPMV_F(coo_heavy_min) TSPMV_F(coo_piece) TSPMV_F(strip_even) TSPMV_F(wg_strips)
         TSPMV_F(x_window) TSPMV_F(x_stride1) TSPMV_F(x_stride2) TSPMV_F(mv_native) TSPMV_F(mv_xcd_chunk) TSPMV_F(lds_pad) TSPMV_F(y_store)
-        TSPMV_F(desc_dict) TSPMV_F(nt_stream) TSPMV_F(x_panel_kb) TSPMV_F(x_panel_merge) TSPMV_F(placement_tries) TSPMV_F(x_slice_passes) TSPMV_F(deterministic) TSPMV_F(absorb) TSPMV_F(value_narrow) TSPMV_F(reserved)
+        TSPMV_F(desc_dict) TSPMV_F(nt_stream) TSPMV_F(x_panel_kb) TSPMV_F(x_panel_merge) TSPMV_F(placement_tries) TSPMV_F(x_slice_passes) TSPMV_F(deterministic) TSPMV_F(absorb) TSPMV_F(value_narrow) TSPMV_F(unit_lean) TSPMV_F(reserved)
 #undef TSPMV_F
         return o;
     }();
@@ -380,6 +382,7 @@
         const bool flip = ms2[1] > 0 && ms2[1] < ms2[0] * 0.985;
         best->st.nt_stream = flip ? 1 - rule : rule;
         best->info[TILESPMV_INFO_NT_STREAM] = best->st.nt_stream;
+        best->info[TILESPMV_INFO_UNIT_LEAN] = unit_lean_form(best->st, best->entry_mode, best->wg_strips);
         if (ms2[flip ? 1 : 0] > 0) best_ms = std::min(best_ms, ms2[flip ? 1 : 0]);
     }
     if (best) {
@@ -718,6 +721,7 @@
     I[TILESPMV_INFO_NUM_TASKS] = n_tasks; I[TILESPMV_INFO_NUM_SPLIT_ROWS] = (long long)fix.size();
     I[TILESPMV_INFO_FALLBACK_NNZ] = f_nnz;
     I[TILESPMV_INFO_UNIT_VALUE_BYTES] = plan->st.uval_narrow == 2 ? 2 : plan->st.uval_narrow ? 4 : sv;
+    I[TILESPMV_INFO_UNIT_LEAN] = plan->kernel == TILESPMV_KERNEL_STREAM ? unit_lean_form(plan->st, plan->entry_mode, plan->wg_strips) : 0;
     if (plan->kernel != TILESPMV_KERNEL_STREAM) { I[TILESPMV_INFO_ENTRY_ORDERED] = 1; I[TILESPMV_INFO_STRIP_COST] = target; }
     I[TILESPMV_INFO_BUILD_US] = (long long)(now_us() - t_create0) - I[TILESPMV_INFO_UPLOAD_US];
     I[TILESPMV_INFO_STREAM_BYTES] = model_bytes + (long long)colA * sv + (long long)rows * sv +
diff --git a/tilespmv_amd/csrc/hip_plan_device.h b/tilespmv_amd/csrc/hip_plan_device.h
--- a/tilespmv_amd/csrc/hip_plan_device.h
+++ b/tilespmv_amd/csrc/hip_plan_device.h
@@ -26,6 +26,7 @@
 int dev_pack_desc(const uint4 *d_udesc, const uint2 *d_urow, const uint4 *d_ucol, const int4 *d_map, int ntasks, UDesc *d_packed, URow *d_packed_row, uint4 *d_packed_col);
 int dev_all_narrowable(const val_t *d_uval, long long n, bool *all_float, bool *all_half);
 int dev_shift_histogram(const UDesc *d_packed, long long NUP, unsigned long long hist[8]);
+int dev_count_flag(const UDesc *d_packed, long long NUP, unsigned flag, long long *count);
 struct DictRanges { int off[9]; };
 int dev_dict_patterns(const UDesc *d_packed, long long NUP, size_t cap, std::vector<uint4> &dict, DictRanges *ranges, bool *over);
 int dev_compact_desc(const UDesc *d_packed, long long NUP, const uint4 *d_dict, DictRanges ranges, int cb_bits, unsigned *d_compact);
diff --git a/tilespmv_amd/csrc/hip_plan_device.hip b/tilespmv_amd/csrc/hip_plan_device.hip
--- a/tilespmv_amd/csrc/hip_plan_device.hip
+++ b/tilespmv_amd/csrc/hip_plan_device.hip
@@ -629,6 +629,26 @@
     return 0;
 }
 
+__global__ __launch_bounds__(256) void k_pd_count_flag(const UDesc *__restrict__ packed, long long n, unsigned flag, unsigned long long *__restrict__ count)
+{
+    unsigned c = 0;
+    for (long long i = (long long)blockIdx.x * blockDim.x + threadIdx.x; i < n; i += (long long)gridDim.x * blockDim.x) c += ((packed[i].w0 >> UNIT_FLAG_SHIFT) & flag) ? 1u : 0u;
+    if (c) atomicAdd(count, (unsigned long long)c);
+}
+int dev_count_flag(const UDesc *d_packed, long long NUP, unsigned flag, long long *count)
+{
+    *count = 0;
+    if (NUP <= 0) return 0;
+    Tmp<unsigned long long> c;
+    PD_TRY(c.alloc(1, true));
+    hipLaunchKernelGGL(k_pd_count_flag, dim3((unsigned)std::min<long long>(nblk(NUP, 256), 4096)), dim3(256), 0, 0, d_packed, NUP, flag, c.p);
+    PD_TRY(hipGetLastError());
+    unsigned long long h = 0;
+    PD_TRY(hipMemcpy(&h, c.p, sizeof(h), hipMemcpyDeviceToHost));
+    *count = (long long)h;
+    return 0;
+}
+
 int dev_shift_histogram(const UDesc *d_packed, long long NUP, unsigned long long hist[8])
 {
     for (int c = 0; c < 8; c++) hist[c] = 0;
diff --git a/tilespmv_amd/csrc/hip_plan_internal.h b/tilespmv_amd/csrc/hip_plan_internal.h
--- a/tilespmv_amd/csrc/hip_plan_internal.h
+++ b/tilespmv_amd/csrc/hip_plan_internal.h
@@ -58,6 +58,7 @@
     int placement_tries;
     int deterministic;
     int absorb;
+    int unit_lean;
     int value_narrow;
     bool value_map;
     int desc_dict;
diff --git a/tilespmv_amd/csrc/hip_plan_stream.hip b/tilespmv_amd/csrc/hip_plan_stream.hip
--- a/tilespmv_amd/csrc/hip_plan_stream.hip
+++ b/tilespmv_amd/csrc/hip_plan_stream.hip
@@ -109,6 +109,7 @@
     long long value_bytes() const { return narrow == 2 ? 2 : narrow ? 4 : sv; }
     long long value_group() const { return narrow ? UNIT_GROUP_NARROW : UNIT_GROUP; }
     void choose_value_width();
+    void set_unit_facts(long long nrowunit, long long nderived) { S.unit_facts = (nrowunit == 0 ? UNIT_FACT_NO_ROWUNIT : 0) | (nderived == 0 ? UNIT_FACT_NO_DERIVED : 0); }
     int reserve_values()
     {
         if (narrow == 2) return plan->reserve((size_t)NUP * 16, reinterpret_cast<const unsigned short **>(&S.uval));
@@ -713,6 +714,11 @@
     }
     plan->info[TILESPMV_INFO_DESC_BYTES] = desc_bytes();
     if (rc == 0 && !pooled) { unsigned long long hist[8]; if (dev_shift_histogram(d_packed, NUP, hist) != 0) rc = -3; else plan->info[TILESPMV_INFO_DERIVED_UNITS] = (long long)hist[UNIT_DERIVED_CODE]; }
+    if (rc == 0 && !pooled) {
+        long long nrowunit = 0;
+        if (dev_count_flag(d_packed, NUP, UNIT_ROWUNIT, &nrowunit) != 0) rc = -3;
+        else set_unit_facts(nrowunit, plan->info[TILESPMV_INFO_DERIVED_UNITS]);
+    }
     rc |= reserve_values();
     if (rc == 0) {
         e = launch_pair_values(d_uval, const_cast<val_t *>(S.uval), (const int4 *)d_map, (int)pair_map.size(), narrow);
@@ -731,6 +737,7 @@
     choose_value_width();
     if (rc) return;
     S.uval_narrow = narrow;
+    S.unit_facts = 0; S.unit_lean = K.unit_lean;
     if (narrow == 2) plan->size_hint -= std::min(plan->size_hint, (size_t)(NU * 16 * (sv - value_bytes())));
     const long long G = value_group();
     auto padded = [&](long long n) { return (n + G - 1) / G * G; };
@@ -892,7 +899,12 @@
             rc |= plan->upload(dict.data(), dict.size(), &S.udict);
         } else rc |= plan->upload(packed.data(), (size_t)NUP, &S.udesc);
         plan->info[TILESPMV_INFO_DESC_BYTES] = desc_bytes();
-        if (!pooled) { long long nder = 0; for (long long u = 0; u < NUP; u++) nder += (packed[(size_t)u].w0 >> UNIT_SHIFT_SHIFT) == UNIT_DERIVED_CODE; plan->info[TILESPMV_INFO_DERIVED_UNITS] = nder; }
+        if (!pooled) {
+            long long nder = 0, nrowunit = 0;
+            for (long long u = 0; u < NUP; u++) { nder += (packed[(size_t)u].w0 >> UNIT_SHIFT_SHIFT) == UNIT_DERIVED_CODE; nrowunit += ((packed[(size_t)u].w0 >> UNIT_FLAG_SHIFT) & UNIT_ROWUNIT) != 0; }
+            plan->info[TILESPMV_INFO_DERIVED_UNITS] = nder;
+            set_unit_facts(nrowunit, nder);
+        }
         if (pooled && !wide && !pool_dict) rc |= plan->upload(packed_row.data(), (size_t)NUP, &S.urow);
         if (wide) rc |= plan->upload(packed_col.data(), (size_t)NUP, &S.ucol);
         if (on_device) {
diff --git a/tilespmv_amd/csrc/hip_units_kernel.h b/tilespmv_amd/csrc/hip_units_kernel.h
--- a/tilespmv_amd/csrc/hip_units_kernel.h
+++ b/tilespmv_amd/csrc/hip_units_kernel.h
@@ -204,18 +204,29 @@
 }
 
 extern __shared__ __attribute__((aligned(16))) unsigned char s_dyn[];
-#if defined(UNITS_KERNEL) != defined(UNITS_NARROW_FORM)
-#error "hip_units_kernel.h: define UNITS_KERNEL and UNITS_NARROW_FORM together (or neither: k_units, floats)"
-#endif
-#ifndef UNITS_KERNEL
+#if defined(UNITS_LEAN) ? (!defined(UNITS_KERNEL) || defined(UNITS_NARROW_FORM)) : (defined(UNITS_KERNEL) != defined(UNITS_NARROW_FORM))
+#error "hip_units_kernel.h: define UNITS_KERNEL and UNITS_NARROW_FORM together (or neither: k_units, floats); UNITS_LEAN goes with UNITS_KERNEL alone (the value form is a template argument there)"
+#endif
+#if !defined(UNITS_KERNEL) && !defined(UNITS_LEAN)
 #define UNITS_KERNEL k_units
 #define UNITS_NARROW_FORM 1
 #endif
+#ifdef UNITS_LEAN
+template <int UB, int ECOO, int GPB, bool CD, bool NTS, int VF, bool DERIVED>
+__global__ __launch_bounds__(16 * GPB, UNITS_MIN_WAVES) void UNITS_KERNEL(DevStream S, int rowA, int colA, int xcd_chunk, val_t *__restrict__ partial,
+                                               const val_t *__restrict__ x, val_t *__restrict__ y)
+{
+    constexpr bool LEAN = true, POOL = false, WIDE = false, NARROW = VF != 0, ROWUNITS = false;
+    constexpr int VFORM = VF;
+    static_assert(ECOO != 1 && GPB == 16 && NTS && VF >= 0 && VF <= (sizeof(val_t) == 8 ? 2 : 0), "lean forms: entry mode 0 / 2, 16 strips, nontemporal streams, a value form of this build");
+#else
 template <int UB, int ECOO, int GPB, bool CD, bool NTS, bool POOL = false, bool WIDE = false, bool NARROW = false>
 __global__ __launch_bounds__(16 * GPB, ECOO == 1 ? 4 : ECOO == 2 ? (POOL ? POOL_ECOO2_MIN_WAVES : NARROW && UNITS_NARROW_FORM == 2 ? UNITS_MIN_WAVES : ECOO2_MIN_WAVES) : POOL ? (WIDE ? 6 : POOL_MIN_WAVES) : UNITS_MIN_WAVES) void UNITS_KERNEL(DevStream S, int rowA, int colA, int xcd_chunk, val_t *__restrict__ partial,
                                                const val_t *__restrict__ x, val_t *__restrict__ y)
 {
+    constexpr bool LEAN = false, ROWUNITS = true, DERIVED = true;
     constexpr int VFORM = NARROW ? UNITS_NARROW_FORM : 0;
+#endif
     static_assert(VFORM >= 0 && VFORM <= 2, "UNITS_NARROW_FORM: 1 or 2");
     static_assert(!NARROW || (sizeof(val_t) == 8 && !POOL && ECOO != 1 && GPB == 16 && NTS), "narrow values: fp64 classic plans, entry mode 0 / 2, 16 strips, nontemporal streams");
     constexpr int G = NARROW ? UNIT_GROUP_NARROW : UNIT_GROUP;
@@ -353,8 +364,8 @@
 #pragma unroll
         for (int k = 0; k < UB; k++) {
             const unsigned fl = d[k].x >> 24;
-            const unsigned nib = (fl & UNIT_ROWUNIT) ? (unsigned)r : (d[k].y >> (28 - 4 * (r & 7))) & 15u;
-            if ((d[k].x >> UNIT_SHIFT_SHIFT) == UNIT_DERIVED_CODE && r != 15) xv[k] = 0;
+            const unsigned nib = (ROWUNITS && (fl & UNIT_ROWUNIT)) ? (unsigned)r : (d[k].y >> (28 - 4 * (r & 7))) & 15u;
+            if (DERIVED && (d[k].x >> UNIT_SHIFT_SHIFT) == UNIT_DERIVED_CODE && r != 15) { if constexpr (!LEAN) xv[k] = 0; }
             else if constexpr (UNIT_X32) xv[k] = x[x_index32(unit_x_base32(d[k].x), nib, xlast32)];
             else xv[k] = x[min(unit_x_base(d[k].x) + nib, xlast)];
         }
@@ -369,7 +380,7 @@
             for (int k = 0; k < nrows; k++) s_y[g][k][r] = 0;
             wave_lds_fence();
         }
-        constexpr bool LATE_PROLOGUE = VFORM == 2;
+        constexpr bool LATE_PROLOGUE = VFORM == 2 || LEAN;
         if constexpr (!LATE_PROLOGUE) unit_prologue();
         if (wr.y > wr.x) {
             int ge = wr.y;
@@ -466,9 +477,11 @@
             else atomicAdd(&s_y[g][0][0] + dest, (lacc_t)prod);
             return;
         }
-        if (flags & UNIT_ROWUNIT) {
-            prod = strip_allreduce(prod);
-            if (r != (int)(word1 & 15u)) prod = 0;
+        if constexpr (ROWUNITS) {
+            if (flags & UNIT_ROWUNIT) {
+                prod = strip_allreduce(prod);
+                if (r != (int)(word1 & 15u)) prod = 0;
+            }
         }
         acc += prod;
         if (flags & UNIT_EOR) {
@@ -492,6 +505,53 @@
         }
         int chunk_end = unit_begin + DCHUNK;
         val_t xprev = 0;
+        if constexpr (LEAN) {
+            const grp_t *vnext = ugrp + (long long)(unit_begin + UB) * (16 / G);
+            auto batch = [&](const int u, auto tail) {
+#pragma clang fp contract(off)
+                constexpr bool TAIL = decltype(tail)::value;
+                if (u == chunk_end) {
+                    wave_lds_fence();
+                    if constexpr (CD) s_d[g][r] = udesc_expand(S, dnext.x, make_uint4(dnext.y, dnext.w, dnext.z, 0u));
+                    else s_d[g][r] = udesc_park_form(dnext);
+                    wave_lds_fence();
+                    chunk_end += DCHUNK;
+                    if constexpr (CD) {
+                        const uint4 p = udict_of(S, wnn);
+                        dnext = make_uint4(wnn, p.x, p.z, p.y);
+                        wnn = stream_load<NT_DESC>(udw + (min(chunk_end + DCHUNK + r + 1, unit_end) - 1));
+                    } else dnext = load_udesc_raw(S.udesc, min(chunk_end + r + 1, unit_end) - 1);
+                }
+                fetch_batch(u - (chunk_end - DCHUNK));
+                sval_t vn[UB];
+                if constexpr (!TAIL) {
+#pragma unroll
+                    for (int k = 0; k < UB; k += G) {
+                        const grp_t *pa = vnext + k * (16 / G);
+                        if constexpr (UNIT_TAIL_HOT) pa = (u + UB + k < unit_end) ? pa : reinterpret_cast<const grp_t *>(S.uval);
+                        else pa = ugrp + (long long)min(u + UB + k, last_grp) * (16 / G);
+                        const grp_t pv = stream_load<NT>(pa);
+#pragma unroll
+                        for (int q = 0; q < G; q++) vn[k + q] = pv[q];
+                    }
+                    vnext += UB * (16 / G);
+                }
+                __builtin_amdgcn_sched_barrier(0);
+#pragma unroll
+                for (int k = 0; k < UB; k++) {
+                    val_t xu = xv[k];
+                    if constexpr (DERIVED) { xu = unit_x_use(xv[k], xprev, d[k].x, r); xprev = xu; }
+                    if (!TAIL || u + k < unit_end) retire(v[k] * xu, d[k].x >> 24, d[k].y);
+                }
+                if constexpr (!TAIL) {
+#pragma unroll
+                    for (int k = 0; k < UB; k++) v[k] = vn[k];
+                }
+            };
+            int u = unit_begin;
+            for (; u + UB <= unit_end; u += UB) batch(u, std::false_type());
+            if (u < unit_end) batch(u, std::true_type());
+        } else
         for (int u = unit_begin; u < unit_end; u += UB) {
             if (u == chunk_end) {
                 wave_lds_fence();
```
